# dmuley/sph-code

Hardware: AMD Instinct MI355X
Metric: particle-steps/sec + achieved HBM GB/s, 10^6-particle 3D sphere, 1/2/4/8 GPUs (higher is better)
Workload: dtype f64

## Files before the change

### include/sphx.h

```cpp
#ifndef SPHX_H
#define SPHX_H

#include <stddef.h>
#include <stdint.h>

#ifdef __cplusplus
extern "C" {
#endif

#define SPHX_OK            0
#define SPHX_E_ARG        -1
#define SPHX_E_HIP        -2
#define SPHX_E_NOMEM      -3
#define SPHX_E_STATE      -4

#define SPHX_MAX_K        64
#define SPHX_MAX_SPECIES  32

typedef struct sphx_ctx sphx_ctx;

typedef struct sphx_constants {
    double k_B;
    double amu;
    double m_h;
    double m_0;
    double dt_0;
    double max_age;
    double pos_clamp;
    double solar_luminosity;
    double c;
} sphx_constants;

typedef struct sphx_stats {
    double ms_grid;
    double ms_search;
    double ms_prep;
    double ms_density;
    double ms_pi;
    double ms_visc;
    double ms_integrate;
    double ms_total;
    int64_t n;
    int64_t steps;
    int64_t candidates;
    int64_t retries;
    int64_t cells;
    int64_t refresh_steps;
    int64_t rebuild_steps;
    double  cell_size;
    double  ms_gravity;
    int64_t fallback_queries;
    double  ms_species;
    int64_t short_rows;
    int64_t detail_steps;
    int64_t far_queries;
    int64_t outlier_levels;
    int64_t bad_accel;
    int64_t bad_energy;
    int64_t bad_state;
    int64_t bad_h;
    int64_t search_steps;
    int64_t tie_entries;
    int64_t tie_capacity;
    int64_t visc_blobs_settled;
    int64_t pi_waves_settled;
} sphx_stats;

int         sphx_create(sphx_ctx** out, int device);
void        sphx_destroy(sphx_ctx* ctx);
const char* sphx_last_error(const sphx_ctx* ctx);
int         sphx_version(void);
const char* sphx_build_info(void);
const char* sphx_tunables(const sphx_ctx* ctx);
int sphx_selftest_scan(sphx_ctx* ctx, int n, unsigned seed, long long* mismatches, int* single_launch);
int sphx_selftest_grid_order(sphx_ctx* ctx, int n, const double* x, const double* y, const double* z, double cell_size,
                             long long* mismatches, int* new_chain_taken);
int sphx_selftest_mfma_cull(sphx_ctx* ctx, double E, int blocks, unsigned seed, double* max_err_over_E2,
                            double* wrong_signs, double* kappa);
int         sphx_host_alloc(void** out, size_t bytes);
int         sphx_host_free(void* p);
int         sphx_set_constants(sphx_ctx* ctx, const sphx_constants* c);
int         sphx_get_constants(const sphx_ctx* ctx, sphx_constants* c);
int         sphx_set_tuning(sphx_ctx* ctx, double rscale, double cell_factor);
int         sphx_set_timing_detail(sphx_ctx* ctx, int on);
int         sphx_set_incremental(sphx_ctx* ctx, int verlet, double rscale_build);

int sphx_neighbors(sphx_ctx* ctx, int64_t n, int k, const double* points, double dist,
                   double eps, int64_t* idx, double* dist_out, int64_t* nontriv, double* h);

int sphx_hydro_update(sphx_ctx* ctx, int64_t n, int k, int s, const int64_t* neighbor,
                      const double* points, const double* mass, const double* sizes,
                      const double* f_un, const double* particle_type, const double* T,
                      const double* mu_array, const double* gamma_array,
                      const double* velocities, int visc_mode,
                      double* hydro_accel, double* visc_accel, double* visc_heat,
                      double* rho, double* nden, double* f_un_nb, double* rho_dust);

int sphx_density(sphx_ctx* ctx, int64_t n, int k, const double* points, const double* mass,
                 const double* particle_type, const int64_t* neighbor, double d, double* out);
int sphx_dust_density(sphx_ctx* ctx, int64_t n, int k, const double* points, const double* mass,
                      const int64_t* neighbor, const double* particle_type, const double* sizes,
                      double* out);
int sphx_num_dens(sphx_ctx* ctx, int64_t n, int k, const double* mass, const double* points,
                  const double* mu_array, const int64_t* neighbor, double d, double* out);
int sphx_del_pressure(sphx_ctx* ctx, int64_t n, int k, const double* points, const double* mass,
                      const double* particle_type, const int64_t* neighbor,
                      const double* E_internal, const double* gamma_array, double d,
                      double* out );
int sphx_artificial_viscosity(sphx_ctx* ctx, int64_t n, int k, const int64_t* neighbor,
                              const double* points, const double* particle_type,
                              const double* sizes, const double* mass, const double* densities,
                              const double* velocities, const double* T,
                              const double* gamma_array, const double* mu_array, double d,
                              double* visc_accel , double* visc_heat );
int sphx_crossing_time(sphx_ctx* ctx, int64_t n, int k, const int64_t* neighbor,
                       const double* velocities, const double* sizes,
                       const double* particle_type, double* out );
int sphx_net_impulse(sphx_ctx* ctx, int64_t n, int k, const double* points, const double* mass,
                     const double* sizes, const double* velocities, const double* particle_type,
                     const int64_t* neighbor, const double* mean_grain_mass,
                     const double* mean_cross, double* accel_onto ,
                     double* accel_reaction );

int sphx_gravity_direct(sphx_ctx* ctx, int64_t n, const double* mass, const double* points,
                        const double* sizes, double softening, double G, double* accel);

int sphx_gravity_tree(sphx_ctx* ctx, int64_t n, const double* mass, const double* points,
                      const double* sizes, double softening, double G, int ws, int k_cells,
                      double* accel);

int sphx_gravity_tree_parts(sphx_ctx* ctx, int64_t n, const double* mass, const double* points,
                            const double* sizes, double softening, double G, int ws, int k_cells, int nparts,
                            const int32_t* part_of, double* accel, int64_t* counts);

int sphx_agb_yields(sphx_ctx* ctx, int64_t n, const double* masses, const double* metallicities,
                    int nspl, const int32_t* ntx, const int32_t* nty, const double* tx,
                    const double* ty, const double* coeffs, const int32_t* mapto, double divisor,
                    int nspecies, const double* mu_specie, const double* composition,
                    double solar_mass, double* dust_out ,
                    double* gas_out );

int sphx_dt_rule(sphx_ctx* ctx, int64_t n, const double* ct, const int32_t* first, double* dt);
int sphx_clamp_arrays(sphx_ctx* ctx, int64_t n, double* points, double* velocities);
int sphx_leapfrog(sphx_ctx* ctx, int64_t n, double* points, double* velocities, double* total_accel,
                  const double* old_accel, double* E_internal, double* T, const double* mass,
                  const double* mu, const double* gamma, const double* ptype, const double* grav_accel,
                  const double* delp, const double* densities, const double* dust_densities,
                  const double* drag_on_gas, const double* drag_reaction, const double* av_accel,
                  const double* av_heat, double dt);

int sphx_state_upload(sphx_ctx* ctx, int64_t n, int s, const double* pos, const double* vel,
                      const double* mass, const double* ptype, const double* f_un,
                      const double* T, const double* mu, const double* gamma,
                      const double* E_internal, const double* accel_old);
int sphx_state_set_drag(sphx_ctx* ctx, const double* mean_grain_mass, const double* mean_cross);
int sphx_state_set_agb(sphx_ctx* ctx, int nspl, const int32_t* ntx, const int32_t* nty, const double* tx,
                       const double* ty, const double* coeffs, const int32_t* mapto, double divisor,
                       const double* mu_specie, double solar_mass);
int sphx_state_download_species(sphx_ctx* ctx, double* F, double* Z, double* agb_dust);
int sphx_state_set_loop_forms(sphx_ctx* ctx, int on, double d);
int sphx_set_clip_grad(sphx_ctx* ctx, int on);
int sphx_set_visc_mode(sphx_ctx* ctx, int mode);
int sphx_state_set_gravity(sphx_ctx* ctx, int mode, double G);
int sphx_set_gravity_order(sphx_ctx* ctx, int order);
int sphx_step(sphx_ctx* ctx, int nsteps, int k, double dist, int first, double fixed_dt);
int sphx_state_download(sphx_ctx* ctx, double* pos, double* vel, double* accel,
                        double* E_internal, double* T, double* sizes, double* rho,
                        double* nden, double* visc_heat, double* dt_last);
int sphx_state_download_pressure(sphx_ctx* ctx, double* pressure);
int sphx_arb_fields(sphx_ctx* ctx, int64_t n, const double* points, const double* mass,
                    const double* particle_type, const double* sizes, const double* T, const double* n_part,
                    const double* value, double d, int64_t m, const double* arb_points, double radius,
                    double* density, double* dust_density, double* temperature, double* dust_temperature,
                    double* photoionization, int64_t* count, int64_t* candidates, int64_t ball_id);
int sphx_arb_fields_list(sphx_ctx* ctx, int64_t n, const double* points, const double* mass,
                         const double* particle_type, const double* sizes, const double* T, const double* n_part,
                         const double* value, double d, int64_t m, const double* arb_points,
                         const int64_t* row_start, const int64_t* members, double* density, double* dust_density,
                         double* temperature, double* dust_temperature, double* photoionization, int64_t* count,
                         int64_t* candidates);
int sphx_state_sample(sphx_ctx* ctx, double d, const double* n_part, const double* value, int64_t m,
                      const double* arb_points, double radius, double* density, double* dust_density,
                      double* temperature, double* dust_temperature, double* photoionization, int64_t* count,
                      int64_t* candidates);
int sphx_arb_last_timing(sphx_ctx* ctx, double ms[4]);
#define SPHX_RAD_LINE        0
#define SPHX_RAD_SEGMENT     1
#define SPHX_RAD_TILE        256
#define SPHX_RAD_WG_RAYS     256
#define SPHX_RAD_SRC_CHUNK   16
int sphx_rad_columns(sphx_ctx* ctx, int64_t n, const double* points, const double* sizes, const double* mass,
                     const double* mu, const double* cross, int64_t n_src, const double* src, int64_t n_dst,
                     const double* dst, int mode, double* blocked , double* star_distance );
int sphx_rad_transfer(sphx_ctx* ctx, int64_t n, const double* points, const double* ptypes, const double* mass,
                      const double* sizes, const double* cross, const double* mu, int64_t n_src, const double* src,
                      const double* luminosities, int64_t n_dst, const double* dst, double dt, int mode, double* lf2,
                      double* momentum, double* extinction, double* blocked, double* star_distance, double* lum_factor);
int sphx_state_rad_transfer(sphx_ctx* ctx, const double* cross, int64_t n_src, const double* src,
                            const double* luminosities, int64_t n_dst, const double* dst, double dt, int mode, double* lf2,
                            double* momentum, double* extinction, double* blocked, double* star_distance,
                            double* lum_factor);
int sphx_rad_last_timing(sphx_ctx* ctx, double ms[4]);
#define SPHX_COOL_WG         256
int sphx_rad_cooling(sphx_ctx* ctx, int64_t n, int k, int s, const double* points, const double* ptype,
                     const double* mass, const double* f_un, const int64_t* neighbor, const double* mu, const double* T,
                     double dt, double d, double* final_comp, double* energy, double* rec_array,
                     double* row_table );
int sphx_cool_last_timing(sphx_ctx* ctx, double ms[4]);
#define SPHX_DUST_WG              256
#define SPHX_DUST_GUARD_COUNT     0
#define SPHX_DUST_GUARD_FRACTION  1
int sphx_supernova_destruction(sphx_ctx* ctx, int64_t n, int k, int s, const double* points, const double* velocities,
                               const int64_t* neighbor, const double* mass, const double* f_un, const double* mu,
                               const double* sizes, const double* densities, const double* ptype, double crit_mass,
                               double critical_density, const int32_t* species_curve ,
                               const double knots_v[8], const double knots_c[8], const double knots_si[8], int guard_mode,
                               double* frac_destruction, double* frac_reuptake, int64_t* counts );
int sphx_dust_last_timing(sphx_ctx* ctx, double ms[4]);
// ... 106 lines not shown
```

### sph-code_amd/_lib.py

```python
import ctypes as C
import os
import threading
import weakref

import numpy as np

HERE = os.path.dirname(os.path.abspath(__file__))
LIB_PATH = os.environ.get("SPHX_LIB") or os.path.join(HERE, "libsphx.so")

c_double_p = C.POINTER(C.c_double)
c_int64_p = C.POINTER(C.c_int64)
c_int32_p = C.POINTER(C.c_int32)


class SphxConstants(C.Structure):
    _fields_ = [(n, C.c_double) for n in ("k_B", "amu", "m_h", "m_0", "dt_0", "max_age", "pos_clamp", "solar_luminosity",
                                          "c")]


class SphxStats(C.Structure):
    _fields_ = [(n, C.c_double) for n in ("ms_grid", "ms_search", "ms_prep", "ms_density", "ms_pi",
                                          "ms_visc", "ms_integrate", "ms_total")] + \
               [(n, C.c_int64) for n in ("n", "steps", "candidates", "retries", "cells", "refresh_steps",
                                         "rebuild_steps")] + \
               [("cell_size", C.c_double), ("ms_gravity", C.c_double), ("fallback_queries", C.c_int64),
                ("ms_species", C.c_double), ("short_rows", C.c_int64), ("detail_steps", C.c_int64), ("far_queries", C.c_int64),
                ("outlier_levels", C.c_int64), ("bad_accel", C.c_int64), ("bad_energy", C.c_int64), ("bad_state", C.c_int64),
                ("bad_h", C.c_int64), ("search_steps", C.c_int64), ("tie_entries", C.c_int64), ("tie_capacity", C.c_int64),
                ("visc_blobs_settled", C.c_int64), ("pi_waves_settled", C.c_int64)]

    def as_dict(self):
        return {n: getattr(self, n) for n, _ in self._fields_}


SPHX_E_STATE = -4
_P = C.c_void_p
_D = c_double_p
_I = c_int64_p
SIGNATURES = {
    "sphx_create": (C.c_int, [C.POINTER(_P), C.c_int]),
    "sphx_destroy": (None, [_P]),
    "sphx_last_error": (C.c_char_p, [_P]),
    "sphx_version": (C.c_int, []),
    "sphx_build_info": (C.c_char_p, []),
    "sphx_tunables": (C.c_char_p, [_P]),
    "sphx_selftest_scan": (C.c_int, [_P, C.c_int, C.c_uint, C.POINTER(C.c_longlong), C.POINTER(C.c_int)]),
    "sphx_selftest_grid_order": (C.c_int, [_P, C.c_int, _D, _D, _D, C.c_double, C.POINTER(C.c_longlong), C.POINTER(C.c_int)]),
    "sphx_selftest_mfma_cull": (C.c_int, [_P, C.c_double, C.c_int, C.c_uint, _D, _D, _D]),
    "sphx_host_alloc": (C.c_int, [C.POINTER(_P), C.c_size_t]),
    "sphx_host_free": (C.c_int, [_P]),
    "sphx_set_constants": (C.c_int, [_P, C.POINTER(SphxConstants)]),
    "sphx_get_constants": (C.c_int, [_P, C.POINTER(SphxConstants)]),
    "sphx_set_tuning": (C.c_int, [_P, C.c_double, C.c_double]),
    "sphx_set_incremental": (C.c_int, [_P, C.c_int, C.c_double]),
    "sphx_neighbors": (C.c_int, [_P, C.c_int64, C.c_int, _D, C.c_double, C.c_double, _I, _D, _I, _D]),
    "sphx_hydro_update": (C.c_int, [_P, C.c_int64, C.c_int, C.c_int, _I] + [_D] * 9 + [C.c_int] + [_D] * 7),
    "sphx_density": (C.c_int, [_P, C.c_int64, C.c_int, _D, _D, _D, _I, C.c_double, _D]),
    "sphx_dust_density": (C.c_int, [_P, C.c_int64, C.c_int, _D, _D, _I, _D, _D, _D]),
    "sphx_num_dens": (C.c_int, [_P, C.c_int64, C.c_int, _D, _D, _D, _I, C.c_double, _D]),
    "sphx_del_pressure": (C.c_int, [_P, C.c_int64, C.c_int, _D, _D, _D, _I, _D, _D, C.c_double, _D]),
    "sphx_artificial_viscosity": (C.c_int, [_P, C.c_int64, C.c_int, _I] + [_D] * 9 + [C.c_double, _D, _D]),
    "sphx_crossing_time": (C.c_int, [_P, C.c_int64, C.c_int, _I, _D, _D, _D, _D]),
    "sphx_net_impulse": (C.c_int, [_P, C.c_int64, C.c_int, _D, _D, _D, _D, _D, _I, _D, _D, _D, _D]),
    "sphx_agb_yields": (C.c_int, [_P, C.c_int64, _D, _D, C.c_int, C.POINTER(C.c_int32), C.POINTER(C.c_int32), _D, _D, _D,
                                  C.POINTER(C.c_int32), C.c_double, C.c_int, _D, _D, C.c_double, _D, _D]),
    "sphx_dt_rule": (C.c_int, [_P, C.c_int64, _D, C.POINTER(C.c_int32), _D]),
    "sphx_clamp_arrays": (C.c_int, [_P, C.c_int64, _D, _D]),
    "sphx_leapfrog": (C.c_int, [_P, C.c_int64] + [_D] * 18 + [C.c_double]),
    "sphx_state_upload": (C.c_int, [_P, C.c_int64, C.c_int] + [_D] * 10),
    "sphx_state_set_drag": (C.c_int, [_P, _D, _D]),
    "sphx_state_set_agb": (C.c_int, [_P, C.c_int, C.POINTER(C.c_int32), C.POINTER(C.c_int32), _D, _D, _D,
                                     C.POINTER(C.c_int32), C.c_double, _D, C.c_double]),
    "sphx_state_download_species": (C.c_int, [_P, _D, _D, _D]),
    "sphx_state_set_loop_forms": (C.c_int, [_P, C.c_int, C.c_double]),
    "sphx_set_clip_grad": (C.c_int, [_P, C.c_int]),
    "sphx_set_visc_mode": (C.c_int, [_P, C.c_int]),
    "sphx_state_set_gravity": (C.c_int, [_P, C.c_int, C.c_double]),
    "sphx_set_gravity_order": (C.c_int, [_P, C.c_int]),
    "sphx_gravity_direct": (C.c_int, [_P, C.c_int64, _D, _D, _D, C.c_double, C.c_double, _D]),
    "sphx_gravity_tree": (C.c_int, [_P, C.c_int64, _D, _D, _D, C.c_double, C.c_double, C.c_int, C.c_int, _D]),
    "sphx_gravity_tree_parts": (C.c_int, [_P, C.c_int64, _D, _D, _D, C.c_double, C.c_double, C.c_int, C.c_int, C.c_int,
                                          c_int32_p, _D, _I]),
    "sphx_step": (C.c_int, [_P, C.c_int, C.c_int, C.c_double, C.c_int, C.c_double]),
    "sphx_state_download": (C.c_int, [_P] + [_D] * 10),
    "sphx_state_download_pressure": (C.c_int, [_P, _D]),
    "sphx_arb_fields": (C.c_int, [_P, C.c_int64] + [_D] * 7 + [C.c_double, C.c_int64, _D, C.c_double] + [_D] * 5 + [_I, _I, C.c_int64]),
    "sphx_arb_last_timing": (C.c_int, [_P, _D]),
    "sphx_arb_fields_list": (C.c_int, [_P, C.c_int64] + [_D] * 7 + [C.c_double, C.c_int64, _D, _I, _I] + [_D] * 5 + [_I, _I]),
    "sphx_state_sample": (C.c_int, [_P, C.c_double, _D, _D, C.c_int64, _D, C.c_double] + [_D] * 5 + [_I, _I]),
    "sphx_rad_columns": (C.c_int, [_P, C.c_int64] + [_D] * 5 + [C.c_int64, _D, C.c_int64, _D, C.c_int, _D, _D]),
    "sphx_rad_transfer": (C.c_int, [_P, C.c_int64] + [_D] * 6 + [C.c_int64, _D, _D, C.c_int64, _D, C.c_double, C.c_int] + [_D] * 6),
    "sphx_state_rad_transfer": (C.c_int, [_P, _D, C.c_int64, _D, _D, C.c_int64, _D, C.c_double, C.c_int] + [_D] * 6),
    "sphx_rad_last_timing": (C.c_int, [_P, _D]),
    "sphx_rad_cooling": (C.c_int, [_P, C.c_int64, C.c_int, C.c_int] + [_D] * 4 + [_I, _D, _D, C.c_double, C.c_double] + [_D] * 4),
    "sphx_cool_last_timing": (C.c_int, [_P, _D]),
    "sphx_supernova_destruction": (C.c_int, [_P, C.c_int64, C.c_int, C.c_int, _D, _D, _I] + [_D] * 6 + [C.c_double, C.c_double,
                                             c_int32_p, _D, _D, _D, C.c_int, _D, _D, _I]),
    "sphx_dust_last_timing": (C.c_int, [_P, _D]),
    "sphx_chemisputtering_2": (C.c_int, [_P, C.c_int64, C.c_int, C.c_int, _D, _I] + [_D] * 6 + [C.c_double, C.c_double] + [_D] * 4 +
                                         [C.c_double] * 3 + [_D, _D, _I]),
    "sphx_chem_last_timing": (C.c_int, [_P, _D]),
    "sphx_dust_bookkeeping": (C.c_int, [_P, C.c_int64, C.c_int] + [_D] * 8 + [C.c_double] + [_D] * 5 + [_I]),
    "sphx_state_dust_phase": (C.c_int, [_P, C.c_double, C.c_double] + [_D] * 5 + [C.c_double] * 5 + [c_int32_p, _D, _D, _D, C.c_int] +
                                        [_D] * 7 + [_I, _I, _D, _I]),
    "sphx_phase_last_timing": (C.c_int, [_P, _D]),
    "sphx_state_download_neighbors": (C.c_int, [_P, _I]),
    "sphx_state_download_composition": (C.c_int, [_P, _D, _D, _D, _D]),
    "sphx_state_download_drag": (C.c_int, [_P, _D, _D]),
    "sphx_get_stats": (C.c_int, [_P, C.POINTER(SphxStats)]),
    "sphx_reset_stats": (C.c_int, [_P]),
    "sphx_set_stream": (C.c_int, [_P, C.c_void_p]),
    "sphx_reset_stream": (C.c_int, [_P]),
    "sphx_sync": (C.c_int, [_P]),
    "sphx_dev_set_mean_h": (C.c_int, [_P, C.c_double]),
    "sphx_dev_search": (C.c_int, [_P, C.c_int64, C.c_int64, C.c_int, _P, _P, C.c_double, C.c_double, _P]),
    "sphx_dev_get_order": (C.c_int, [_P, C.c_int64, _P]),
    "sphx_dev_prep": (C.c_int, [_P] + [_P] * 8),
    "sphx_dev_density": (C.c_int, [_P] + [_P] * 4),
    "sphx_dev_pi": (C.c_int, [_P] + [_P] * 4),
    "sphx_dev_visc": (C.c_int, [_P] + [_P] * 4),
    "sphx_dev_visc_pairwise": (C.c_int, [_P] + [_P] * 5),
    "sphx_dev_clamp": (C.c_int, [_P, C.c_int64, _P, _P]),
    "sphx_dev_pack_rows": (C.c_int, [_P, C.c_int64, _P, C.c_int, C.POINTER(C.c_void_p), C.POINTER(C.c_int32), _P]),
    "sphx_dev_regroup": (C.c_int, [_P, C.c_int64, _P, C.c_int64, _P, C.c_int, C.POINTER(C.c_void_p),
                                   C.POINTER(C.c_int32), C.POINTER(C.c_void_p)]),
    "sphx_dev_need_map": (C.c_int, [_P, C.c_int64, _P, _P, C.POINTER(C.c_double), C.c_double, C.c_int, _P]),
    "sphx_dev_integrate_auto": (C.c_int, [_P, C.c_int64] + [_P] * 13 + [C.c_int, C.c_double, _P]),
    "sphx_dev_reach": (C.c_int, [_P, C.c_int64, _P, _P, C.c_double, C.c_double, C.c_double, _P]),
    "sphx_set_timing_detail": (C.c_int, [_P, C.c_int]),
    "sphx_dev_reach_dt": (C.c_int, [_P, C.c_int64, _P, _P, C.c_double, C.c_double, _P, _P]),
    "sphx_dev_plan_mask": (C.c_int, [_P, C.c_int64, _P, C.POINTER(C.c_double), C.c_double, C.c_int, C.c_int, C.c_int, _P, _P, _P]),
    "sphx_dev_step_scalars": (C.c_int, [_P, C.c_int64, _P, _P, C.c_double, C.c_double, _P, _P]),
    "sphx_dev_integrate": (C.c_int, [_P, C.c_int64] + [_P] * 12 + [C.c_double]),
    "sphx_dev_drag": (C.c_int, [_P] + [_P] * 6),
    "sphx_dev_set_drag_terms": (C.c_int, [_P] + [_P] * 4),
    "sphx_dev_gravity_build": (C.c_int, [_P, C.c_int64, C.c_int64, _P, _P, _D]),
    "sphx_dev_gravity_local": (C.c_int, [_P, C.c_int, C.c_double, _P, C.c_double, _P]),
    "sphx_dev_gravity_export": (C.c_int, [_P, C.c_int, C.c_int, _P, C.c_int, _P, C.c_int64, _P, C.c_int64, _P]),
    "sphx_dev_gravity_remote": (C.c_int, [_P, C.c_int64, _P, _P, C.c_int64, _P, C.c_int64, C.c_double, _P, C.c_double, _P]),
    "sphx_dev_set_gravity_accel": (C.c_int, [_P, _P]),
    "sphx_dev_set_agb": (C.c_int, [_P, C.c_int, C.c_int, C.POINTER(C.c_int32), C.POINTER(C.c_int32), _D, _D, _D,
                                   C.POINTER(C.c_int32), C.c_double, _D, C.c_double]),
    "sphx_dev_species": (C.c_int, [_P, C.c_int] + [_P] * 5),
    "sphx_dev_loop_prep": (C.c_int, [_P] + [_P] * 8 + [C.c_double]),
    "sphx_dev_loop_pass1": (C.c_int, [_P] + [_P] * 5),
    "sphx_dev_loop_pass2": (C.c_int, [_P] + [_P] * 4),
    "sphx_dev_loop_pass2_interior": (C.c_int, [_P]),
    "sphx_dev_set_reach_cap": (C.c_int, [_P, C.c_double]),
    "sphx_dev_select_blobs": (C.c_int, [_P, C.c_int]),
    "sphx_dev_blob_split_counts": (C.c_int, [_P, _P]),
    "sphx_dev_integrate_loop": (C.c_int, [_P, C.c_int64] + [_P] * 14 + [C.c_int, C.c_double, C.c_double, _P]),
}

_lib = None
_lock = threading.Lock()


def load_library():
    global _lib
    with _lock:
        if _lib is not None:
            return _lib
        if not os.path.exists(LIB_PATH):
            raise RuntimeError(
                "libsphx.so is not built (%s). Run `python -c 'import __graft_entry__ as g; g.build()'` "
                "or `python sph-code_amd/build.py`. There is no CPU fallback." % LIB_PATH)
        lib = C.CDLL(LIB_PATH)
        for name, (res, args) in SIGNATURES.items():
            fn = getattr(lib, name)
            fn.restype = res
            fn.argtypes = args
        _lib = lib
        return lib


def f64(a, shape=None):
    out = np.ascontiguousarray(a, dtype=np.float64)
    if shape is not None and out.shape != shape:
        raise ValueError("expected shape %s, got %s" % (shape, out.shape))
    return out


# ... 132 lines not shown
```

### sph-code_amd/csrc/sphx_api.hip

```cpp
#include "sphx_internal.h"
#include <stdarg.h>
#include <stdlib.h>
#include <new>

int sphx_set_err(sphx_ctx* ctx, int code, const char* fmt, ...) {
    if (ctx) {
        va_list ap;
        va_start(ap, fmt);
        vsnprintf(ctx->err, sizeof(ctx->err), fmt, ap);
        va_end(ap);
    }
    return code;
}

void sphx_release(sphx_ctx* ctx, DevBuf& b) {
    for (size_t q = 0; q < ctx->allocs.size(); ++q)
        if (ctx->allocs[q] == b.p) { ctx->allocs[q] = ctx->allocs.back(); ctx->allocs.pop_back(); break; }
    if (b.p) (void)hipFree(b.p);
    b.p = nullptr;
    b.cap = 0;
}

int sphx_ensure(sphx_ctx* ctx, DevBuf& b, size_t bytes, hipStream_t in_use_on) {
    if (bytes == 0) bytes = 8;
// ... 495 lines not shown
static int step_cell_hint(sphx_ctx* ctx, int64_t n, double* cell_hint) {
    *cell_hint = 0.0;
    if (ctx->step_count == 0) return SPHX_OK;
    const double* hs;
    if (ctx->lag_hvalid[ctx->lag_hslot]) {
        HIPCHK(hipEventSynchronize(ctx->lag_halias[ctx->lag_hslot] ? ctx->lag_halias[ctx->lag_hslot]
                                                                     : ctx->lag_hev[ctx->lag_hslot]));
        hs = ctx->pinned->lag[ctx->lag_hslot].hs;
        const u64* sv = (const u64*)hs;
        for (int q = 0; q < 10; ++q) ctx->knn_lag[q] = sv[(SC_NFAILQ - SC_HSUM) + q];
        ctx->knn_lag_valid = true;
    } else {
        HIPCHK(hipMemcpyAsync(ctx->pinned->hsum, ctx->scal.as<double>() + SC_HSUM, sizeof(ctx->pinned->hsum),
                              hipMemcpyDeviceToHost, ctx->stream));
        HIPCHK(hipStreamSynchronize(ctx->stream));
        hs = ctx->pinned->hsum;
    }
    const double hmean = hs[3] > 0.0 ? hs[0] / hs[3] : 0.0;
    if (hmean > 0.0 && isfinite(hmean)) {
        *cell_hint = ctx->cell_factor * sphx_cell_feedback(ctx, n) * hmean;
        ctx->h_clip = ctx->h_clip_factor * hmean;
    }
    return SPHX_OK;
}

static int step_search(sphx_ctx* ctx, int k, double dist, hipEvent_t* ev) {
    const int64_t n = ctx->n;
    if (ctx->use_verlet) SPHX_TRY(sphx_clamp(ctx, n, ctx->st));
    SPHX_TRY(sphx_ensure(ctx, ctx->nbr, (size_t)k * ctx->npad * sizeof(int)));
    if (ctx->use_verlet && ctx->list_valid && ctx->list_n == n && ctx->list_k == k) {
        StateArrays& r = ctx->st;
        HIPCHK(hipEventRecord(ev[1], ctx->stream));
        int64_t nfail = 0;
        SPHX_TRY(sphx_knn_refresh(ctx, n, k, r.x.as<double>(), r.y.as<double>(), r.z.as<double>(),
                                  ctx->nbr.as<int>(), r.hprev.as<double>(), &nfail));
        if (nfail == 0) {
            ctx->stats.refresh_steps++;
            return SPHX_OK;
        }
        ctx->list_valid = false;
    }
    double cell_hint = 0.0;
    SPHX_TRY(step_cell_hint(ctx, n, &cell_hint));
    {
        StateArrays& r = ctx->st;
        const bool blob = ctx->use_blob && !ctx->use_verlet;
        GridBuildOpts g;
        g.lagged = true;
        g.alias_ev = ev[1];
        g.sort_cells_later = blob;
        g.count_curve = blob && ctx->side_stream && ctx->ev_perm;
        if (!ctx->use_verlet) { g.clamp_vel[0] = r.vx.as<double>(); g.clamp_vel[1] = r.vy.as<double>(); g.clamp_vel[2] = r.vz.as<double>(); }
        SPHX_TRY(sphx_build_grid(ctx, n, k, r.x.as<double>(), r.y.as<double>(), r.z.as<double>(), cell_hint, g));
        if (blob) SPHX_TRY(sphx_build_blob_order(ctx, n, true));
    }
    const bool split = ctx->side_stream && !ctx->use_verlet;
    SPHX_TRY(sphx_permute_state(ctx, n, split, ev[1]));
    StateArrays& r = ctx->st;
    KnnIn in;
    in.xs = r.x.as<double>(); in.ys = r.y.as<double>(); in.zs = r.z.as<double>();
    in.id = r.id.as<int>(); in.inv = ctx->inv.as<int>();
    in.rsearch = r.hprev.as<double>();
    in.hinted = ctx->step_count > 0 && !ctx->use_verlet;
    in.lag_external = true;
    in.rscale = ctx->rscale;
    in.rbound = dist;
    KnnOut o;
    o.nbr = ctx->nbr.as<int>();
    o.h_sorted = r.hprev.as<double>();
    o.idx64 = nullptr; o.dist = nullptr; o.nontriv = nullptr; o.h_by_id = nullptr;
    if (ctx->use_verlet) {
        SPHX_TRY(sphx_ensure(ctx, ctx->list64, (size_t)n * 64 * sizeof(int)));
        SPHX_TRY(sphx_ensure(ctx, ctx->dref, (size_t)n * sizeof(double)));
        o.list64 = ctx->list64.as<int>();
        o.dref = ctx->dref.as<double>();
        in.rscale = ctx->rscale_build;
    }
    SPHX_TRY(sphx_knn(ctx, n, k, in, o));
    if (split) HIPCHK(hipStreamWaitEvent(ctx->stream, ctx->ev_perm, 0));
    if (ctx->use_verlet) {
        SPHX_TRY(sphx_save_list_positions(ctx, n, r.x.as<double>(), r.y.as<double>(), r.z.as<double>()));
        ctx->list_valid = true;
        ctx->list_n = n;
        ctx->list_k = k;
    }
    ctx->stats.rebuild_steps++;
    return SPHX_OK;
}

static int step_h_sums_out(sphx_ctx* ctx, int64_t n, const double* h, hipStream_t stream) {
    SPHX_TRY(sphx_hsum(ctx, n, h, stream));
    const int hsl = ctx->lag_hslot ^ 1;
    HIPCHK(hipMemcpyAsync(ctx->pinned->lag[hsl].hs, ctx->scal.as<double>() + SC_HSUM,
                          (SC_KGDBG + 2 - SC_HSUM + 1) * sizeof(double), hipMemcpyDeviceToHost, stream));
    HIPCHK(hipEventRecord(ctx->lag_hev[hsl], stream));
    ctx->lag_halias[hsl] = nullptr;
    ctx->lag_hvalid[hsl] = true;
    ctx->lag_hslot = hsl;
    return SPHX_OK;
}

static int step_sums(sphx_ctx* ctx, int k, hipEvent_t* ev, hipEvent_t search_end, bool detail) {
    const int64_t n = ctx->n;
    StateArrays& s = ctx->st;
    const bool pairwise = ctx->visc_mode == 1 && !ctx->loop_forms;
    const bool fork = ctx->qorder && ctx->use_lds && !ctx->loop_forms && ctx->side_stream;
    if (fork) HIPCHK(hipStreamWaitEvent(ctx->side_stream, search_end, 0));
    else SPHX_TRY(step_h_sums_out(ctx, n, s.hprev.as<double>(), ctx->stream));
    if (ctx->qorder && ctx->use_lds) SPHX_TRY(sphx_blob_translate(ctx, n, k));
    const bool species = ctx->s > 0 && ctx->fun_id.p;
    if (ctx->loop_forms) {
        if (ctx->drag || species)
            SPHX_TRY(sphx_prep(ctx, n, prep_in_of_state(s), pairwise, ctx->stream));
        if (detail) HIPCHK(hipEventRecord(ev[3], ctx->stream));
        SPHX_TRY(sphx_loop_step_sums(ctx, n, k, ctx->loop_d));
        if (detail) HIPCHK(hipEventRecord(ev[9], ctx->stream));
        if (species) SPHX_TRY(sphx_step_species(ctx, n, k));
        if (detail) HIPCHK(hipEventRecord(ev[4], ctx->stream));
        if (detail) HIPCHK(hipEventRecord(ev[5], ctx->stream));
    } else {
        SPHX_TRY(sphx_prep(ctx, n, prep_in_of_state(s), pairwise, fork ? ctx->side_stream : ctx->stream));
        if (fork) {
            HIPCHK(hipEventRecord(ctx->ev_join, ctx->side_stream));
            HIPCHK(hipStreamWaitEvent(ctx->stream, ctx->ev_join, 0));
            SPHX_TRY(step_h_sums_out(ctx, n, s.hprev.as<double>(), ctx->side_stream));
        }
        if (detail) HIPCHK(hipEventRecord(ev[3], ctx->stream));
        const bool sp_fused = species && ctx->species_fused && ctx->species_lds && ctx->use_lds && ctx->qorder && ctx->blob_lists &&
                              !ctx->map_perm && ctx->sp == 16 && ctx->s <= 16 && k <= SPHX_MAX_K;
        if (sp_fused) {
            const int S = ctx->s;
            SPHX_TRY(sphx_ensure(ctx, ctx->rho, (size_t)n * sizeof(double)));
            SPHX_TRY(sphx_ensure(ctx, ctx->rhod, (size_t)n * sizeof(double)));
            SPHX_TRY(sphx_ensure(ctx, ctx->nden, (size_t)n * sizeof(double)));
            SPHX_TRY(sphx_ensure(ctx, ctx->G, (size_t)n * 3 * sizeof(double)));
            SPHX_TRY(sphx_ensure(ctx, ctx->ha, (size_t)n * 3 * sizeof(double)));
            SPHX_TRY(sphx_ensure(ctx, ctx->F, (size_t)n * S * sizeof(double)));
            if (ctx->agb_on) {
                SPHX_TRY(sphx_ensure(ctx, ctx->Zmet, (size_t)n * sizeof(double)));
                SPHX_TRY(sphx_ensure(ctx, ctx->agb_dust, (size_t)n * S * sizeof(double)));
            }
            SPHX_TRY(sphx_blob_density_species(ctx, n, k, true, S, ctx->fun_id.as<double>(), s.id.as<int>(),
                                               s.m.as<double>(), ctx->F.as<double>(), ctx->Zmet.as<double>(),
                                               ctx->agb_dust.as<double>(), (ctx->agb_on && ctx->Zmet.p && ctx->agb_dust.p) ? 1 : 0));
        } else {
            SPHX_TRY(sphx_pass_density(ctx, n, k, true));
        }
        if (detail) HIPCHK(hipEventRecord(ev[9], ctx->stream));
        if (species && !sp_fused) SPHX_TRY(sphx_step_species(ctx, n, k));
        if (detail) HIPCHK(hipEventRecord(ev[4], ctx->stream));
        if (ctx->visc_mode == 1) {
            SPHX_TRY(sphx_pass_visc_pw(ctx, n, k, s.m.as<double>()));
        } else {
            SPHX_TRY(sphx_pass_pi(ctx, n, k, s.hprev.as<double>(), s.ptype.as<double>()));
            if (detail) HIPCHK(hipEventRecord(ev[5], ctx->stream));
            SPHX_TRY(sphx_pass_visc(ctx, n, k, s.m.as<double>()));
        }
    }
    if (ctx->drag)
        SPHX_TRY(sphx_pass_drag(ctx, n, k, s.m.as<double>(), s.ptype.as<double>(), s.mgm.as<double>(), s.mcs.as<double>()));
    return SPHX_OK;
}

static int one_step(sphx_ctx* ctx, int k, double dist, int first, double fixed_dt, bool call_first, bool call_last) {
    const int64_t n = ctx->n;
    const int ring = (int)(ctx->step_count % 3);
    hipEvent_t* ev = ctx->evring[ring];
    const bool detail = ctx->timing_detail;
    ctx->ev_detail[ring] = detail;
    const bool rec0 = detail || call_first, rec7 = detail || call_last;
    ctx->ev_has07[ring] = (rec0 ? 1 : 0) | (rec7 ? 2 : 0) | (ctx->visc_mode == 1 && !ctx->loop_forms ? 4 : 0);
    ctx->map_perm = nullptr;
    ctx->qorder = nullptr;
    ctx->blob_lists = false;
    ctx->blob_split_valid = false;
    ctx->pass_part = 0;
    ctx->nbr_api_valid = false;
    sphx_step_list_drop(ctx);
    if (rec0) HIPCHK(hipEventRecord(ev[0], ctx->stream));
    SPHX_TRY(step_search(ctx, k, dist, ev));
    HIPCHK(hipEventRecord(ev[2], ctx->stream));
    SPHX_TRY(step_sums(ctx, k, ev, ev[2], detail));
    if (detail) HIPCHK(hipEventRecord(ev[6], ctx->stream));
    StateArrays& s = ctx->st;
    if (ctx->gravity) {
        SPHX_TRY(sphx_ensure(ctx, ctx->grav, (size_t)n * 3 * sizeof(double)));
        double* eps = ctx->scal.as<double>() + SC_GRAV_EPS;
        SPHX_TRY(sphx_median(ctx, n, s.hprev.as<double>(), eps));
        if (ctx->gravity == 1)
            SPHX_TRY(sphx_gravity_launch(ctx, n, s.x.as<double>(), s.y.as<double>(), s.z.as<double>(), 1,
                                         s.m.as<double>(), eps, 0.0, ctx->grav_G, nullptr, ctx->grav.as<double>()));
        else
            SPHX_TRY(sphx_gravity_tree_launch(ctx, n, s.x.as<double>(), s.y.as<double>(), s.z.as<double>(),
                                              s.m.as<double>(), ctx->grav_ws, eps, 0.0, ctx->grav_G, nullptr,
                                              ctx->grav.as<double>()));
    }
    if (detail) HIPCHK(hipEventRecord(ev[8], ctx->stream));
    SPHX_TRY(sphx_integrate(ctx, n, 1, first, fixed_dt));
    if (rec7) HIPCHK(hipEventRecord(ev[7], ctx->stream));
    ctx->step_count++;
    return SPHX_OK;
}

static int collect_stats(sphx_ctx* ctx, int ring) {
    if (!(ctx->ev_pending & (1u << ring))) return SPHX_OK;
    ctx->ev_pending &= ~(1u << ring);
    hipEvent_t* ev = ctx->evring[ring];
    const int has = ctx->ev_has07[ring];
    HIPCHK(hipEventSynchronize((has & 2) ? ev[7] : ev[2]));
    sphx_stats& st = ctx->stats;
    float ms[7] = {0.f, 0.f, 0.f, 0.f, 0.f, 0.f, 0.f};
    HIPCHK(hipEventElapsedTime(&ms[1], ev[1], ev[2]));
    st.ms_search += ms[1];
    st.steps += 1;
    st.search_steps += 1;
    st.n = ctx->n;
    if (!ctx->ev_detail[ring]) return SPHX_OK;
    float tot;
    HIPCHK(hipEventElapsedTime(&tot, ev[0], ev[7]));
    HIPCHK(hipEventElapsedTime(&ms[0], ev[0], ev[1]));
    st.ms_grid += ms[0]; st.ms_total += tot;
    for (int i = 2; i < 6; ++i) {
        if ((has & 4) && i >= 4) break;
        HIPCHK(hipEventElapsedTime(&ms[i], ev[i], ev[i + 1]));
    }
    if (has & 4) HIPCHK(hipEventElapsedTime(&ms[5], ev[4], ev[6]));
    st.ms_prep += ms[2];
    float mg = 0.f, mi = 0.f;
    HIPCHK(hipEventElapsedTime(&mg, ev[6], ev[8]));
    HIPCHK(hipEventElapsedTime(&mi, ev[8], ev[7]));
    ms[6] = mi;
    st.ms_gravity += mg;
    {
        float md = 0.f, msp = 0.f;
        HIPCHK(hipEventElapsedTime(&md, ev[3], ev[9]));
        HIPCHK(hipEventElapsedTime(&msp, ev[9], ev[4]));
        ms[3] = md;
        st.ms_species += msp;
    }
    st.ms_density += ms[3]; st.ms_pi += ms[4]; st.ms_visc += ms[5]; st.ms_integrate += ms[6];
    st.detail_steps += 1;
    return SPHX_OK;
}

extern "C" int sphx_step(sphx_ctx* ctx, int nsteps, int k, double dist, int first, double fixed_dt) {
    if (!ctx) return SPHX_E_ARG;
    if (!ctx->has_state) return sphx_set_err(ctx, SPHX_E_STATE, "sphx_step before sphx_state_upload");
    if (k < 1 || k > SPHX_MAX_K) return sphx_set_err(ctx, SPHX_E_ARG, "N_NEIGH=%d not in 1..%d", k, SPHX_MAX_K);
    if (nsteps < 1) return sphx_set_err(ctx, SPHX_E_ARG, "nsteps=%d < 1", nsteps);
    HIPCHK(hipSetDevice(ctx->device));
    if (!(dist > 0.0) || !isfinite(dist)) dist = 0.0;
    ctx->k = k;
    const bool per_call = !ctx->timing_detail;
    if (per_call) HIPCHK(hipEventRecord(ctx->ev[8], ctx->stream));
    for (int it = 0; it < nsteps; ++it) {
        const int ring = (int)(ctx->step_count % 3);
        SPHX_TRY(collect_stats(ctx, ring));
        SPHX_TRY(one_step(ctx, k, dist, first && it == 0, fixed_dt, false, false));
        ctx->ev_pending |= 1u << ring;
        SPHX_TRY(collect_stats(ctx, (ring + 1) % 3));
    }
    ctx->step_list_valid = true; ctx->step_qorder = ctx->qorder; ctx->step_list_n = ctx->n; ctx->step_list_k = k;
    if (per_call) HIPCHK(hipEventRecord(ctx->ev[9], ctx->stream));
    HIPCHK(hipMemcpyAsync(ctx->pinned->scal, ctx->scal.p, SC_NSLOTS * 8, hipMemcpyDeviceToHost, ctx->stream));
    HIPCHK(hipStreamSynchronize(ctx->stream));
    for (int r = 0; r < 3; ++r) SPHX_TRY(collect_stats(ctx, (int)((ctx->step_count + r) % 3)));
    if (per_call) {
        float tot = 0.f;
        HIPCHK(hipEventElapsedTime(&tot, ctx->ev[8], ctx->ev[9]));
        ctx->stats.ms_total += tot;
    }
    const u64* sc = ctx->pinned->scal;
    memcpy(&ctx->dt_last, &sc[SC_DT], sizeof(double));
    ctx->stats.candidates = (int64_t)sc[SC_CAND];
    ctx->stats.retries = (int64_t)sc[SC_RETRY];
    ctx->stats.fallback_queries = (int64_t)(u32)sc[SC_NFAILQ];
    ctx->stats.short_rows = (int64_t)sc[SC_SHORT];
    SPHX_TRY(sphx_badc_read(ctx));
    return SPHX_OK;
}

extern "C" int sphx_state_download(sphx_ctx* ctx, double* pos, double* vel, double* accel,
                                   double* E_internal, double* T, double* sizes, double* rho,
                                   double* nden, double* visc_heat, double* dt_last) {
    if (!ctx) return SPHX_E_ARG;
    if (!ctx->has_state) return sphx_set_err(ctx, SPHX_E_STATE, "no state uploaded");
    HIPCHK(hipSetDevice(ctx->device));
    const int64_t n = ctx->n;
    const size_t nb = (size_t)n * sizeof(double);
    StateArrays& s = ctx->st;
    const int* id = s.id.as<int>();
    SPHX_TRY(sphx_ensure(ctx, ctx->out_a, 3 * nb));
    double* stage = ctx->out_a.as<double>();
    struct V3 { double* host; DevBuf *a, *b, *c; };
    V3 v3[] = {{pos, &s.x, &s.y, &s.z}, {vel, &s.vx, &s.vy, &s.vz}, {accel, &s.ax, &s.ay, &s.az}};
    for (V3& v : v3) {
        if (!v.host) continue;
        SPHX_TRY(sphx_soa3_to_aos_by_id(ctx, n, id, v.a->as<double>(), v.b->as<double>(), v.c->as<double>(), stage));
        SPHX_TRY(download(ctx, v.host, stage, 3 * nb));
        HIPCHK(hipStreamSynchronize(ctx->stream));
    }
    struct V1 { double* host; const double* dev; };
    const bool stepped = ctx->step_count > 0;
    V1 v1[] = {{E_internal, s.E.as<double>()}, {T, s.T.as<double>()}, {sizes, s.hprev.as<double>()},
               {rho, stepped ? ctx->rho.as<double>() : nullptr},
               {nden, stepped ? ctx->nden.as<double>() : nullptr},
               {visc_heat, stepped ? ctx->vh.as<double>() : nullptr}};
    for (V1& v : v1) {
        if (!v.host) continue;
        if (!v.dev) { memset(v.host, 0, nb); continue; }
        SPHX_TRY(sphx_scatter_rows_by_id(ctx, n, 1, id, v.dev, stage));
        SPHX_TRY(download(ctx, v.host, stage, nb));
        HIPCHK(hipStreamSynchronize(ctx->stream));
    }
    if (dt_last) *dt_last = ctx->dt_last;
    return SPHX_OK;
}

int sphx_agb_table_set(sphx_ctx* ctx, int S, int nspl, const int32_t* ntx, const int32_t* nty, const double* tx, const double* ty,
                       const double* coeffs, const int32_t* mapto, double divisor, const double* mu_specie, double solar_mass) {
    ctx->agb_on = false;
    if (nspl == 0) return SPHX_OK;
    if (S < 7 || S > AGB_MAX_SPEC) return sphx_set_err(ctx, SPHX_E_ARG, "AGB table: %d species (7..%d)", S, AGB_MAX_SPEC);
    if (!ntx || !nty || !tx || !ty || !coeffs || !mapto || !mu_specie)
        return sphx_set_err(ctx, SPHX_E_ARG, "AGB table: NULL argument");
    if (nspl < 1 || nspl > AGB_MAX_SPL) return sphx_set_err(ctx, SPHX_E_ARG, "AGB table: %d splines", nspl);
    if (!(divisor != 0.0)) return sphx_set_err(ctx, SPHX_E_ARG, "AGB table: divisor is 0");
    HIPCHK(hipSetDevice(ctx->device));
    AgbTable& t = ctx->agb;
    t.nspl = nspl; t.nspec = S;
    size_t ntx_tot = 0, nty_tot = 0, nc_tot = 0;
    for (int o = 0; o < nspl; ++o) {
        if (ntx[o] < 4 || nty[o] < 4) return sphx_set_err(ctx, SPHX_E_ARG, "AGB table: spline %d has fewer than 4 knots", o);
        if (mapto[o] < 0 || mapto[o] >= S) return sphx_set_err(ctx, SPHX_E_ARG, "AGB table: mapto[%d]=%d out of range", o, mapto[o]);
        ntx_tot += ntx[o]; nty_tot += nty[o]; nc_tot += (size_t)(ntx[o] - 2) * (nty[o] - 2);
    }
    size_t ox = 0, oy = ntx_tot, oc = ntx_tot + nty_tot;
    for (int o = 0; o < nspl; ++o) {
        t.tx_off[o] = (int)ox; t.ty_off[o] = (int)oy; t.c_off[o] = (int)oc;
        t.ntx[o] = ntx[o]; t.nty[o] = nty[o]; t.mapto[o] = mapto[o];
        ox += ntx[o]; oy += nty[o]; oc += (size_t)(ntx[o] - 2) * (nty[o] - 2);
    }
    for (int s = 0; s < S; ++s) t.mu[s] = mu_specie[s];
    t.divisor = divisor; t.solar = solar_mass;
    SPHX_TRY(sphx_ensure(ctx, ctx->agb_knots, (ntx_tot + nty_tot + nc_tot + 6 * (size_t)nspl) * sizeof(double)));
    double* kd = ctx->agb_knots.as<double>();
    {
        double meta[6 * AGB_MAX_SPL];
        t.covered = 0u;
        for (int o = 0; o < nspl; ++o) {
            bool later = false;
            for (int o2 = o + 1; o2 < nspl; ++o2) later = later || mapto[o2] == mapto[o];
            meta[6 * o + 0] = t.tx_off[o]; meta[6 * o + 1] = t.ty_off[o]; meta[6 * o + 2] = t.c_off[o];
            meta[6 * o + 3] = t.ntx[o]; meta[6 * o + 4] = t.nty[o]; meta[6 * o + 5] = later ? -1.0 : (double)mapto[o];
            t.covered |= 1u << mapto[o];
        }
        t.meta_off = (int)(ntx_tot + nty_tot + nc_tot);
        HIPCHK(hipMemcpyAsync(kd + t.meta_off, meta, 6 * (size_t)nspl * sizeof(double), hipMemcpyHostToDevice, ctx->stream));
        HIPCHK(hipStreamSynchronize(ctx->stream));
    }
    HIPCHK(hipMemcpyAsync(kd, tx, ntx_tot * sizeof(double), hipMemcpyHostToDevice, ctx->stream));
    HIPCHK(hipMemcpyAsync(kd + ntx_tot, ty, nty_tot * sizeof(double), hipMemcpyHostToDevice, ctx->stream));
    HIPCHK(hipMemcpyAsync(kd + ntx_tot + nty_tot, coeffs, nc_tot * sizeof(double), hipMemcpyHostToDevice, ctx->stream));
    HIPCHK(hipStreamSynchronize(ctx->stream));
    t.knots = kd;
    ctx->agb_on = true;
    return SPHX_OK;
}

extern "C" int sphx_state_set_agb(sphx_ctx* ctx, int nspl, const int32_t* ntx, const int32_t* nty, const double* tx,
                                  const double* ty, const double* coeffs, const int32_t* mapto, double divisor,
                                  const double* mu_specie, double solar_mass) {
    if (!ctx) return SPHX_E_ARG;
    if (!ctx->has_state) return sphx_set_err(ctx, SPHX_E_STATE, "sphx_state_set_agb before sphx_state_upload");
    ctx->agb_on = false;
    if (nspl == 0) return SPHX_OK;
    if (ctx->s < 7 || !ctx->fun_id.p)
        return sphx_set_err(ctx, SPHX_E_STATE, "sphx_state_set_agb: the state carries no composition (f_un) of >= 7 species");
    return sphx_agb_table_set(ctx, ctx->s, nspl, ntx, nty, tx, ty, coeffs, mapto, divisor, mu_specie, solar_mass);
}

__global__ __launch_bounds__(256) void scatter_species_major(int n, int S, const int* id, const double* in, double* out) {
    const int t = blockIdx.x * blockDim.x + threadIdx.x;
    if (t >= n) return;
    const size_t o = (size_t)id[t];
    for (int s = 0; s < S; ++s) out[(size_t)s * n + o] = in[(size_t)s * n + t];
}
extern "C" int sphx_state_download_species(sphx_ctx* ctx, double* F, double* Z, double* agb_dust) {
    if (!ctx) return SPHX_E_ARG;
    if (!ctx->has_state || ctx->s < 1 || !ctx->fun_id.p || ctx->step_count < 1)
        return sphx_set_err(ctx, SPHX_E_STATE, "sphx_state_download_species: no species pass has run (state without f_un, "
                                                 "or no step yet)");
    if ((Z || agb_dust) && !ctx->agb_on) return sphx_set_err(ctx, SPHX_E_STATE, "sphx_state_download_species: no AGB table set");
    HIPCHK(hipSetDevice(ctx->device));
    const int64_t n = ctx->n;
    const int S = ctx->s;
    const int* id = ctx->st.id.as<int>();
    SPHX_TRY(sphx_ensure(ctx, ctx->out_a, (size_t)n * S * sizeof(double)));
    double* stage = ctx->out_a.as<double>();
    if (F) {
        hipLaunchKernelGGL(scatter_species_major, dim3((unsigned)((n + 255) / 256)), dim3(256), 0, ctx->stream, (int)n, S, id,
                           ctx->F.as<double>(), stage);
        SPHX_TRY(download(ctx, F, stage, (size_t)n * S * sizeof(double)));
        HIPCHK(hipStreamSynchronize(ctx->stream));
    }
    if (Z) {
        SPHX_TRY(sphx_scatter_rows_by_id(ctx, n, 1, id, ctx->Zmet.as<double>(), stage));
        SPHX_TRY(download(ctx, Z, stage, (size_t)n * sizeof(double)));
        HIPCHK(hipStreamSynchronize(ctx->stream));
    }
    if (agb_dust) {
        SPHX_TRY(sphx_scatter_rows_by_id(ctx, n, S, id, ctx->agb_dust.as<double>(), stage));
        SPHX_TRY(download(ctx, agb_dust, stage, (size_t)n * S * sizeof(double)));
        HIPCHK(hipStreamSynchronize(ctx->stream));
    }
    return SPHX_OK;
}

int sphx_badc_read(sphx_ctx* ctx) {
    u64* hb = ctx->pinned->badc;
    HIPCHK(hipMemcpyAsync(hb, ctx->badc.p, (size_t)BADC_BUCKETS * BADC_STRIDE * sizeof(u64), hipMemcpyDeviceToHost, ctx->stream));
    HIPCHK(hipStreamSynchronize(ctx->stream));
    u64 tot[4] = {0, 0, 0, 0};
    for (int b = 0; b < BADC_BUCKETS; ++b)
        for (int q = 0; q < 4; ++q) tot[q] += hb[b * BADC_STRIDE + q];
    ctx->stats.bad_accel = (int64_t)tot[BAD_ACCEL]; ctx->stats.bad_energy = (int64_t)tot[BAD_ENERGY];
    ctx->stats.bad_state = (int64_t)tot[BAD_STATE]; ctx->stats.bad_h = (int64_t)tot[BAD_H];
    return SPHX_OK;
}

extern "C" int sphx_get_stats(sphx_ctx* ctx, sphx_stats* out) {
    if (!ctx || !out) return SPHX_E_ARG;
    SPHX_TRY(sphx_dev_collect(ctx));
    if (ctx->map_perm) {
        HIPCHK(hipSetDevice(ctx->device));
        SPHX_TRY(sphx_badc_read(ctx));
    }
    ctx->stats.tie_entries = 0;
    ctx->stats.tie_capacity = ctx->tie_cap_last;
    if (ctx->tie_count_dev) {
        int cnt = 0;
        u64 nfail = 0;
        HIPCHK(hipSetDevice(ctx->device));
        HIPCHK(hipMemcpyAsync(&cnt, ctx->tie_count_dev, sizeof(int), hipMemcpyDeviceToHost, ctx->stream));
        HIPCHK(hipMemcpyAsync(&nfail, ctx->scal.as<u64>() + SC_NFAILQ, sizeof(u64), hipMemcpyDeviceToHost, ctx->stream));
        HIPCHK(hipStreamSynchronize(ctx->stream));
        ctx->stats.tie_entries = (int64_t)(u32)cnt;
        if (ctx->map_perm) ctx->stats.fallback_queries = (int64_t)(u32)nfail;
    }
    if (ctx->scal.p) {
        u64 cnt[2] = {0, 0};
        HIPCHK(hipSetDevice(ctx->device));
        HIPCHK(hipMemcpyAsync(cnt, ctx->scal.as<u64>() + SC_SETTLED, sizeof(cnt), hipMemcpyDeviceToHost, ctx->stream));
        HIPCHK(hipStreamSynchronize(ctx->stream));
        ctx->stats.visc_blobs_settled = (int64_t)cnt[0];
        ctx->stats.pi_waves_settled = (int64_t)cnt[1];
    }
    *out = ctx->stats;
    for (int w = 0; w < 2; ++w) {
        if (!ctx->lbs_state[w].p) continue;
        int flag = 0;
        HIPCHK(hipSetDevice(ctx->device));
        HIPCHK(hipMemcpy(&flag, ctx->lbs_state[w].as<int>() + 2, sizeof(int), hipMemcpyDeviceToHost));
        if (flag) return sphx_set_err(ctx, SPHX_E_STATE, "lookback_scan_kernel: a tile's sum never arrived (results since then are wrong)");
    }
    return SPHX_OK;
}
extern "C" int sphx_set_timing_detail(sphx_ctx* ctx, int on) {
    if (!ctx) return SPHX_E_ARG;
    ctx->timing_detail = on != 0;
    return SPHX_OK;
}

extern "C" int sphx_reset_stats(sphx_ctx* ctx) {
    if (!ctx) return SPHX_E_ARG;
    SPHX_TRY(sphx_dev_collect(ctx));
    memset(&ctx->stats, 0, sizeof(ctx->stats));
    HIPCHK(hipMemsetAsync(ctx->scal.as<u64>() + SC_CAND, 0, 2 * sizeof(u64), ctx->stream));
    HIPCHK(hipMemsetAsync(ctx->scal.as<u64>() + SC_SHORT, 0, sizeof(u64), ctx->stream));
    HIPCHK(hipMemsetAsync(ctx->scal.as<u64>() + SC_SETTLED, 0, 2 * sizeof(u64), ctx->stream));
    HIPCHK(hipMemsetAsync(ctx->badc.p, 0, (size_t)BADC_BUCKETS * BADC_STRIDE * sizeof(u64), ctx->stream));
    HIPCHK(hipStreamSynchronize(ctx->stream));
    return SPHX_OK;
}
```

### sph-code_amd/csrc/sphx_blob.h

```cpp
#pragma once
#include "sphx_internal.h"
#include "sphx_pair.h"
#include "sphx_settled.h"

#ifndef BLOB_P
#define BLOB_P 128
#endif
#define BLOB_T (2 * BLOB_P)
#define LPP SPHX_SUM_PARTS
#define PASS_T (BLOB_P * LPP)
#ifndef BLOB_S
#define BLOB_S 960
#endif
#ifndef DEDUP_PRIO
#define DEDUP_PRIO 2
#endif
#ifndef BLOB_STAGE_PRIO
#define BLOB_STAGE_PRIO 1
#endif
#ifndef PASS_MINW
#define PASS_MINW 4
#endif
#define BLOB_PROBES 96
#define SLOT_NONE 0xFFFFu
// ... 5 lines not shown
__device__ __forceinline__ Q4 lload4(const double2* img, int s, int c2) {
    const double2 lo = img[(2 * c2) * BLOB_S + s];
    const double2 hi = img[(2 * c2 + 1) * BLOB_S + s];
    return Q4{lo.x, lo.y, hi.x, hi.y};
}
struct Q8 { Q4 lo, hi; };
__device__ __forceinline__ Q8 lload8(const double2* img, int s) { return Q8{lload4(img, s, 0), lload4(img, s, 1)}; }
template <class Rec>
__device__ __forceinline__ Q8 gload8(const Rec* r) {
    const double* q = reinterpret_cast<const double*>(r);
    return Q8{gload4(q), gload4(q + 4)};
}
__device__ __forceinline__ double sqrt_mid(double x) {
    const double y = __builtin_amdgcn_rsq(x);
    double g = x * y;
    double h = 0.5 * y;
    const double r = __builtin_fma(-h, g, 0.5);
    g = __builtin_fma(g, r, g);
    h = __builtin_fma(h, r, h);
    const double d0 = __builtin_fma(-g, g, x);
    g = __builtin_fma(d0, h, g);
    const double d1 = __builtin_fma(-g, g, x);
    g = __builtin_fma(d1, h, g);
    return x > 0.0 ? g : 0.0;
}
struct SqrtMid { __device__ __forceinline__ double operator()(double x) const { return sqrt_mid(x); } };

__device__ __forceinline__ double pair_swap(double v) {
    const long long b = __double_as_longlong(v);
    const int lo = __builtin_amdgcn_update_dpp(0, (int)b, 0xB1, 0xF, 0xF, true);
    const int hi = __builtin_amdgcn_update_dpp(0, (int)(b >> 32), 0xB1, 0xF, 0xF, true);
    return __longlong_as_double(((long long)hi << 32) | (unsigned)lo);
}
__device__ __forceinline__ double pair_swap2(double v) {
    const long long b = __double_as_longlong(v);
    const int lo = __builtin_amdgcn_update_dpp(0, (int)b, 0x4E, 0xF, 0xF, true);
    const int hi = __builtin_amdgcn_update_dpp(0, (int)(b >> 32), 0x4E, 0xF, 0xF, true);
    return __longlong_as_double(((long long)hi << 32) | (unsigned)lo);
}
__device__ __forceinline__ double group_total(double acc) {
    acc = acc + pair_swap(acc);
    if (LPP == 4) acc = acc + pair_swap2(acc);
    return acc;
}
__device__ __forceinline__ double group_max(double v) {
    v = fmax(v, pair_swap(v));
    if (LPP == 4) v = fmax(v, pair_swap2(v));
    return v;
}
template <class S>
__device__ __forceinline__ void group_total_fields(S& s) {
    constexpr int NF = sizeof(S) / sizeof(double);
    static_assert(sizeof(S) == NF * sizeof(double), "a struct of doubles");
    double f[NF];
    __builtin_memcpy(f, &s, sizeof(S));
#pragma unroll
    for (int q = 0; q < NF; ++q) f[q] = group_total(f[q]);
    __builtin_memcpy(&s, f, sizeof(S));
}

#define NSTAGE ((BLOB_S + PASS_T - 1) / PASS_T)
#define NB (8 / LPP)
#define KPAD(k) ((((k) + 7) / 8) * 8)
#define IMG_BYTES(per_slot, k) ((size_t)BLOB_S * (per_slot) + (size_t)KPAD(k) * BLOB_P * sizeof(u16))

template <int NSIDE, class Rec>
__device__ __forceinline__ void stage(double2* img, double* side, u16* tile, const Rec* __restrict__ rec,
                                      const double* __restrict__ g0, int g0_stride,
                                      const double* __restrict__ g1, int g1_stride,
                                      const int* __restrict__ uq, const u16* __restrict__ slot16, int npad,
                                      int k, int b) {
    __builtin_amdgcn_s_setprio(BLOB_STAGE_PRIO);
    int ju[NSTAGE];
#pragma unroll
    for (int r = 0; r < NSTAGE; ++r) {
        const int s = threadIdx.x + r * PASS_T;
        ju[r] = (s < BLOB_S) ? uq[s] : -1;
    }
    const int pieces = KPAD(k) * (BLOB_P / 8);
    for (int q = threadIdx.x; q < pieces; q += PASS_T) {
        const int kk = q / (BLOB_P / 8), c = q % (BLOB_P / 8);
        uint4 v = make_uint4(0xFFFFFFFFu, 0xFFFFFFFFu, 0xFFFFFFFFu, 0xFFFFFFFFu);
        if (kk < k) v = *reinterpret_cast<const uint4*>(slot16 + (size_t)kk * npad + (size_t)b * BLOB_P + c * 8);
        *reinterpret_cast<uint4*>(tile + kk * BLOB_P + c * 8) = v;
    }
    double2 c[NSTAGE][4];
    double e0[NSTAGE], e1[NSTAGE];
#pragma unroll
    for (int r = 0; r < NSTAGE; ++r) {
        const int j = ju[r] < 0 ? 0 : ju[r];
        const double2* g = reinterpret_cast<const double2*>(&rec[j]);
        c[r][0] = g[0]; c[r][1] = g[1]; c[r][2] = g[2]; c[r][3] = g[3];
        e0[r] = (NSIDE > 0) ? g0[(size_t)j * g0_stride] : 0.0;
        e1[r] = (NSIDE > 1) ? g1[(size_t)j * g1_stride] : 0.0;
    }
#pragma unroll
    for (int r = 0; r < NSTAGE; ++r) {
        const int s = threadIdx.x + r * PASS_T;
        if (ju[r] >= 0) {
            if (NSIDE == 2) c[r][3].y = e0[r];
            img[0 * BLOB_S + s] = c[r][0]; img[1 * BLOB_S + s] = c[r][1];
            img[2 * BLOB_S + s] = c[r][2]; img[3 * BLOB_S + s] = c[r][3];
            if (NSIDE == 1) side[s] = e0[r];
            if (NSIDE == 2) side[s] = e1[r];
        }
    }
    __builtin_amdgcn_s_setprio(0);
}

__device__ __forceinline__ void load_slots(unsigned (&sl)[NB], const u16* tile, int m0, int half, int t) {
#pragma unroll
    for (int u = 0; u < NB; ++u) sl[u] = tile[(LPP * (m0 + u) + half) * BLOB_P + t];
}
__device__ __forceinline__ bool all_staged(const unsigned (&sl)[NB]) {
    unsigned worst = sl[0];
#pragma unroll
    for (int u = 1; u < NB; ++u) worst = worst > sl[u] ? worst : sl[u];
    return __ballot(worst >= SLOT_OVER) == 0ull;
}


struct BlobSel { const int* list; const int* cnt; int mode; };
__device__ __forceinline__ int blob_sel_count(const BlobSel& s, int nblk) {
    if (!s.list) return nblk;
    return (s.mode == 1) ? s.cnt[0] : (s.mode == 2) ? s.cnt[1] : s.cnt[0] + s.cnt[1];
}
__device__ __forceinline__ int blob_sel_at(const BlobSel& s, int bi, int count) {
    const int q = xcd_block(bi, count);
    return s.list ? s.list[q + (s.mode == 2 ? s.cnt[0] : 0)] : q;
}
BlobSel sphx_blob_sel(sphx_ctx* ctx, int part);

int sphx_blob_grid(sphx_ctx* ctx, int nblk);
int sphx_lds_opt_in(sphx_ctx* ctx, const void* kernel, size_t bytes);

#define BLOB_KERNEL __global__ __launch_bounds__(PASS_T, PASS_MINW) void
#define BLOB_COMMON int n, int npad, int k, int nblk, const int* __restrict__ nbr, const u16* __restrict__ slot16, \
                    const int* __restrict__ uniq, const int* __restrict__ qorder
template <class Kern, class... Rest>
static int blob_launch(sphx_ctx* ctx, Kern kern, int per_slot, size_t extra, int64_t n, int k, Rest... rest) {
    const int64_t npad = sphx_pad64(n);
    const int nblk = (int)((npad + BLOB_P - 1) / BLOB_P);
    SPHX_TRY(sphx_lds_opt_in(ctx, reinterpret_cast<const void*>(kern), IMG_BYTES(per_slot, SPHX_MAX_K) + extra));
    hipLaunchKernelGGL(kern, dim3(sphx_blob_grid(ctx, nblk)), dim3(PASS_T), IMG_BYTES(per_slot, k) + extra, ctx->stream, (int)n,
                       (int)npad, k, nblk, ctx->nbr.as<int>(), ctx->slot16.as<u16>(), ctx->uniq.as<int>(), ctx->qorder, rest...);
    HIPCHK(hipGetLastError());
    return SPHX_OK;
}

template <class P, class = void> struct BlobSettles { static constexpr bool value = false; };
template <class P> struct BlobSettles<P, decltype((void)P::SETTLES)> { static constexpr bool value = P::SETTLES; };
template <class P, class = void> struct BlobSaturates { static constexpr bool value = false; };
template <class P> struct BlobSaturates<P, decltype((void)P::SATURATES)> { static constexpr bool value = P::SATURATES; };
enum { BLOB_CNT_BLOBS_SETTLED = 0, BLOB_CNT_WAVES_SATURATED = 1 };
struct BlobSides { const double* g0 = nullptr; int s0 = 0; const double* g1 = nullptr; int s1 = 0; };

template <int NSIDE>
struct BlobLds {
    static __device__ __forceinline__ double2* img() { extern __shared__ double2 img[]; return img; }
    static __device__ __forceinline__ double* side() { return reinterpret_cast<double*>(img() + 4 * BLOB_S); }
    static __device__ __forceinline__ u16* tile() { return reinterpret_cast<u16*>(side() + (NSIDE ? BLOB_S : 0)); }
};

template <bool FAST, bool CLIP, class P>
__device__ __forceinline__ void blob_batch(const P& ps, typename P::Sums& a, double (&out)[NB], const unsigned (&sl)[NB],
                                           const int* __restrict__ jp, size_t colstep, const typename P::Row& row) {
    typedef BlobLds<P::NSIDE> L;
    typename P::Nb f[NB];
#pragma unroll
    for (int u = 0; u < NB; ++u) {
        if (FAST || sl[u] < SLOT_OVER) f[u] = ps.staged(L::img(), L::side(), (int)sl[u], jp + u * colstep);
        else if (sl[u] == SLOT_OVER) f[u] = ps.global(jp[u * colstep]);
        else f[u] = P::none(row);
    }
    if (FAST) __builtin_amdgcn_sched_barrier(0);
#pragma unroll
    for (int u = 0; u < NB; ++u) {
        out[u] = 0.0;
        if (!FAST && sl[u] == SLOT_NONE) continue;
        out[u] = ps.template term<CLIP>(a, f[u], row);
    }
}
template <class P>
__device__ __forceinline__ void blob_batch_any(const P& ps, int clip, typename P::Sums& a, double (&out)[NB],
                                               const unsigned (&sl)[NB], const int* __restrict__ jp, size_t colstep,
                                               const typename P::Row& row) {
    const bool fast = all_staged(sl);
    if constexpr (P::CLIPS) {
        if (fast && !clip) blob_batch<true, false>(ps, a, out, sl, jp, colstep, row);
        else if (fast) blob_batch<true, true>(ps, a, out, sl, jp, colstep, row);
        else if (!clip) blob_batch<false, false>(ps, a, out, sl, jp, colstep, row);
        else blob_batch<false, true>(ps, a, out, sl, jp, colstep, row);
    } else {
        if (fast) blob_batch<true, false>(ps, a, out, sl, jp, colstep, row);
        else blob_batch<false, false>(ps, a, out, sl, jp, colstep, row);
    }
}
template <bool FAST, class P>
__device__ __forceinline__ void blob_batch_short(const P& ps, double (&out)[NB], const unsigned (&sl)[NB],
                                                 const int* __restrict__ jp, size_t colstep, const typename P::Row& row) {
    typedef BlobLds<P::NSIDE> L;
    typename P::Vel f[NB];
#pragma unroll
    for (int u = 0; u < NB; ++u) {
        if (FAST || sl[u] < SLOT_OVER) f[u] = P::short_staged(L::img(), (int)sl[u]);
        else if (sl[u] == SLOT_OVER) f[u] = ps.short_global(jp[u * colstep]);
        else f[u] = P::short_none(row);
    }
#pragma unroll
    for (int u = 0; u < NB; ++u) {
        out[u] = 0.0;
        if (!FAST && sl[u] == SLOT_NONE) continue;
        out[u] = P::term_short(f[u], row);
    }
}
struct RowAhead { int i, o; unsigned first; double own; };
template <class P>
__device__ __forceinline__ RowAhead blob_row_ahead(const P& ps, int i, int p, int n, const u16* __restrict__ slot16,
                                                   const int* __restrict__ omap) {
    RowAhead r;
    r.i = i;
    r.o = (p < n) ? (omap ? omap[i] : i) : 0x7FFFFFFF;
    r.first = (p < n) ? slot16[p] : SLOT_NONE;
    r.own = ps.own(i);
    return r;
}
template <int T>
__device__ __forceinline__ bool block_all_at_barrier(bool mine, unsigned round) {
    __shared__ int verdict[2][T / 64];
    static_assert(T / 64 == 8, "eight waves: read as two 16-B pieces");
    int* v = verdict[round & 1];
    const int wave_all = __ballot(!mine) == 0ull;
    if ((threadIdx.x & 63) == 0) v[threadIdx.x >> 6] = wave_all;
    __syncthreads();
    const int4 lo = *reinterpret_cast<const int4*>(v), hi = *reinterpret_cast<const int4*>(v + 4);
    const int all = (lo.x & lo.y) & (lo.z & lo.w) & (hi.x & hi.y) & (hi.z & hi.w);
    return __builtin_amdgcn_readfirstlane(all) != 0;
}
template <int T>
__device__ __forceinline__ void block_add_count(unsigned v, u64* dst) {
    __shared__ unsigned sm[T / 64];
    if ((threadIdx.x & 63) == 0) sm[threadIdx.x >> 6] = v;
    __syncthreads();
    if (threadIdx.x == 0) {
        unsigned r = 0;
        for (int w = 0; w < T / 64; ++w) r += sm[w];
        if (r) atomicAdd(dst, (u64)r);
    }
}
template <class P>
__device__ __forceinline__ void blob_row_point(const P& ps, typename P::Row& row, const int* __restrict__ nbr, int p,
                                               int t) {
    typedef BlobLds<P::NSIDE> L;
    const unsigned sl0 = L::tile()[t];
    if (sl0 < SLOT_OVER) P::row_point(row, ps.staged(L::img(), L::side(), (int)sl0, nbr + p));
    else if (sl0 == SLOT_OVER) P::row_point(row, ps.global(nbr[p]));
}

template <class P>
__device__ __forceinline__ void blob_pass(const P& ps, int n, int npad, int k, int nblk, const int* __restrict__ nbr,
                                          const u16* __restrict__ slot16, const int* __restrict__ uniq,
                                          const int* __restrict__ qorder, int clip, const int* __restrict__ omap,
                                          int n_active, u64* ct_bits, const BlobSel& sel, u64* counts = nullptr) {
    static_assert(P::PER_SLOT == 64 + (P::NSIDE ? 8 : 0), "image bytes per slot: the record and one side value");
    constexpr bool SETTLES = BlobSettles<P>::value, SATURATES = BlobSaturates<P>::value;
    static_assert(!SATURATES || LPP == 4, "sphx_wave_saturated: a row's lanes are one nibble of the wave's mask");
    typedef BlobLds<P::NSIDE> L;
    const BlobSides sd = ps.sides();
    const int t = threadIdx.x / LPP, half = threadIdx.x & (LPP - 1);
    u64 my_ct = SPHX_CT_NONE;
    unsigned blobs_settled = 0, waves_saturated = 0;
    const int nsel = blob_sel_count(sel, nblk);
    const int stride = gridDim.x;
    auto particle_of = [&](int bq) -> int {
        const int pq = blob_sel_at(sel, bq, nsel) * BLOB_P + t;
        return (pq < n) ? qorder[pq] : 0;
    };
    auto nothing_left = [&](const RowAhead& r) -> bool {
        return !(r.o < n_active) || sphx_row_settled(r.own, r.first != SLOT_NONE, true);
    };
    RowAhead cur{0, 0x7FFFFFFF, SLOT_NONE, 0.0};
    int i_next = 0;
    bool blob_settled = false;
    unsigned round = 0;
    if constexpr (SETTLES) {
        if ((int)blockIdx.x < nsel)
            cur = blob_row_ahead(ps, particle_of(blockIdx.x), blob_sel_at(sel, blockIdx.x, nsel) * BLOB_P + t, n, slot16, omap);
        if ((int)blockIdx.x + stride < nsel) i_next = particle_of(blockIdx.x + stride);
        blob_settled = block_all_at_barrier<PASS_T>(nothing_left(cur), round++);
    }
    for (int bi = blockIdx.x; bi < nsel; bi += stride) {
        const int b = blob_sel_at(sel, bi, nsel);
        const int p = b * BLOB_P + t;
        int i, o;
        bool settled = false;
        auto fetch_ahead = [&]() {
            if constexpr (SETTLES) {
                if (bi + stride < nsel) {
                    cur = blob_row_ahead(ps, i_next, blob_sel_at(sel, bi + stride, nsel) * BLOB_P + t, n, slot16, omap);
                    if (bi + 2 * stride < nsel) i_next = particle_of(bi + 2 * stride);
                }
            }
        };
        if constexpr (SETTLES) {
            i = cur.i; o = cur.o;
            settled = sphx_row_settled(cur.own, cur.first != SLOT_NONE, o < n_active);
            if (blob_settled) {
                fetch_ahead();
                if (settled && !half) ps.settle(o);
                ++blobs_settled;
                blob_settled = block_all_at_barrier<PASS_T>(nothing_left(cur), round++);
                continue;
            }
        } else {
            i = (p < n) ? qorder[p] : 0;
        }
        stage<P::NSIDE>(L::img(), L::side(), L::tile(), ps.rec, sd.g0, sd.s0, sd.g1, sd.s1, uniq + (size_t)b * BLOB_S,
                        slot16, npad, k, b);
        typename P::Row row = ps.load_row(i);
        if constexpr (!SETTLES) o = (p < n) ? (omap ? omap[i] : i) : 0x7FFFFFFF;
        ps.load_out(row, o, o < n_active);
        if constexpr (SETTLES) fetch_ahead();
        __syncthreads();
        if (o < n_active) {
            if (SETTLES && __ballot(!settled) == 0ull) {
                if constexpr (SETTLES) { if (!half) ps.settle(o); }
            } else {
                if constexpr (P::ROW_FROM_LIST) blob_row_point(ps, row, nbr, p, t);
                typename P::Sums a{};
                double mx = 0.0;
                if (P::wanted(row)) {
                    const int nm = KPAD(k) / LPP;
                    unsigned sl[NB];
                    load_slots(sl, L::tile(), 0, half, t);
                    bool short_form = false;
                    bool short_used = false;
                    for (int m0 = 0; m0 < nm; m0 += NB) {
                        unsigned cur_sl[NB];
#pragma unroll
                        for (int u = 0; u < NB; ++u) cur_sl[u] = sl[u];
                        if (m0 + NB < nm) load_slots(sl, L::tile(), m0 + NB, half, t);
                        double out[NB];
                        const int* jp = nbr + ((size_t)(LPP * m0 + half) * npad + p);
                        if constexpr (SATURATES) {
                            if (__builtin_expect(short_form, false)) {
                                short_used = true;
                                if (all_staged(cur_sl)) blob_batch_short<true>(ps, out, cur_sl, jp, LPP * (size_t)npad, row);
                                else blob_batch_short<false>(ps, out, cur_sl, jp, LPP * (size_t)npad, row);
                            } else {
                                blob_batch_any(ps, clip, a, out, cur_sl, jp, LPP * (size_t)npad, row);
                                short_form = sphx_wave_saturated(__ballot(P::saturated(a)), __ballot(true));
                            }
                        } else {
                            blob_batch_any(ps, clip, a, out, cur_sl, jp, LPP * (size_t)npad, row);
                        }
                        if (P::VOTES) {
#pragma unroll
                            for (int u = 0; u < NB; ++u) mx = fmax(mx, out[u]);
                        }
                    }
                    if (SATURATES && short_used) ++waves_saturated;
                }
                group_total_fields(a);
                if (P::VOTES) mx = group_max(mx);
                if (!half) {
                    const u64 cb = ps.finish(a, mx, row, i, o);
                    my_ct = cb < my_ct ? cb : my_ct;
                }
            }
        }
        if constexpr (SETTLES) blob_settled = block_all_at_barrier<PASS_T>(nothing_left(cur), round++);
        else __syncthreads();
    }
    if (P::VOTES) block_min_vote<PASS_T>(my_ct, ct_bits);
    if constexpr (SETTLES) {
        if (counts && threadIdx.x == 0 && blobs_settled) atomicAdd(counts + BLOB_CNT_BLOBS_SETTLED, (u64)blobs_settled);
    }
    if constexpr (SATURATES) {
        if (counts) block_add_count<PASS_T>(waves_saturated, counts + BLOB_CNT_WAVES_SATURATED);
    }
}
```

### sph-code_amd/csrc/sphx_blob.hip

```cpp
#include "sphx_blob.h"
#include "sphx_wave.h"
#pragma clang fp contract(off)
#include <float.h>
#include <stdlib.h>
#include <stdio.h>
#ifndef BLOB_PI_SATURATES
#define BLOB_PI_SATURATES 1
#endif

#define DD_TAB 2048
#define DD_PROBES 64
__device__ __forceinline__ unsigned dd_hash(int j) { return ((unsigned)j * 2654435761u) >> 21; }

__global__ __launch_bounds__(BLOB_T) void blob_dedup_kernel(int n, int npad, int k, int slots,
                                                            const int* __restrict__ nbr, u16* slot16,
                                                            int* uniq, const int* __restrict__ qorder,
                                                            const int* __restrict__ omap, int n_active,
                                                            unsigned char* bclass) {
    __builtin_amdgcn_s_setprio(DEDUP_PRIO);
    extern __shared__ u16 dd_tile[];
    __shared__ int key[DD_TAB];
    __shared__ u16 slot_of[DD_TAB];
    __shared__ int wave_tot[BLOB_T / 64];
    const int b = xcd_block(blockIdx.x, gridDim.x);
// ... 61 lines not shown
    __syncthreads();
    constexpr int EPT = DD_TAB / BLOB_T;
    const int e0 = threadIdx.x * EPT;
    int cnt = 0;
#pragma unroll
    for (int q = 0; q < EPT; ++q) cnt += key[e0 + q] != -1;
    const int incl = wave_scan_incl(cnt);
    const int lane = threadIdx.x & 63, wv = threadIdx.x >> 6;
    if (lane == 63) wave_tot[wv] = incl;
    __syncthreads();
    int base = incl - cnt, total = 0;
#pragma unroll
    for (int w = 0; w < BLOB_T / 64; ++w) {
        const int tw = wave_tot[w];
        if (w < wv) base += tw;
        total += tw;
    }
    int* uq = uniq + (size_t)b * BLOB_S;
    int needs_ghost = 0;
#pragma unroll
    for (int q = 0; q < EPT; ++q) {
        const int j = key[e0 + q];
        if (j != -1) {
            slot_of[e0 + q] = (u16)(base < slots ? base : SLOT_OVER);
            if (base < slots) uq[base] = j;
            ++base;
            if (bclass && omap[j] >= n_active) needs_ghost = 1;
        }
    }
    for (int q = (total < slots ? total : slots) + threadIdx.x; q < BLOB_S; q += BLOB_T) uq[q] = -1;
    __syncthreads();
    const int pieces = k * (BLOB_P / 8);
    for (int q = threadIdx.x; q < pieces; q += BLOB_T) {
        u16* src = dd_tile + q * 8;
        const int kk = q / (BLOB_P / 8), c = q % (BLOB_P / 8);
        unsigned v[8];
#pragma unroll
        for (int u = 0; u < 8; ++u) {
            const unsigned e = src[u];
            v[u] = e < DD_TAB ? (unsigned)slot_of[e] : e;
            if (v[u] == SLOT_OVER) needs_ghost = 1;
        }
        if ((size_t)b * BLOB_P + c * 8 < (size_t)npad)
            *reinterpret_cast<uint4*>(slot16 + (size_t)kk * npad + (size_t)b * BLOB_P + c * 8) =
                make_uint4(v[0] | (v[1] << 16), v[2] | (v[3] << 16), v[4] | (v[5] << 16), v[6] | (v[7] << 16));
    }
    if (bclass) {
        const int owned_q = (half == 0 && p < n && omap[qorder[p]] < n_active) ? 1 : 0;
        const int any_owned = __syncthreads_or(owned_q);
        const int any_ghost = __syncthreads_or(needs_ghost);
        if (threadIdx.x == 0) bclass[b] = (unsigned char)(!any_owned ? 2 : (any_ghost ? 1 : 0));
    }
}

#define SPLIT_T 1024
__global__ __launch_bounds__(SPLIT_T) void blob_split_kernel(int nblk, const unsigned char* __restrict__ bclass, int* list,
                                                             int* cnt) {
    __shared__ int wsum[2][SPLIT_T / 64];
    const int per = (nblk + SPLIT_T - 1) / SPLIT_T;
    const int b0 = threadIdx.x * per, b1 = (b0 + per < nblk) ? b0 + per : nblk;
    int c0 = 0, c1 = 0;
    for (int b = b0; b < b1; ++b) { const int c = bclass[b]; c0 += c == 0; c1 += c == 1; }
    const int i0 = wave_scan_incl(c0), i1 = wave_scan_incl(c1);
    const int lane = threadIdx.x & 63, wv = threadIdx.x >> 6;
    if (lane == 63) { wsum[0][wv] = i0; wsum[1][wv] = i1; }
    __syncthreads();
    int o0 = i0 - c0, o1 = i1 - c1, t0 = 0, t1 = 0;
    for (int w = 0; w < SPLIT_T / 64; ++w) {
        if (w < wv) { o0 += wsum[0][w]; o1 += wsum[1][w]; }
        t0 += wsum[0][w]; t1 += wsum[1][w];
    }
    for (int b = b0; b < b1; ++b) {
        const int c = bclass[b];
        if (c == 0) list[o0++] = b;
        else if (c == 1) list[t0 + o1++] = b;
    }
    if (threadIdx.x == 0) { cnt[0] = t0; cnt[1] = t1; cnt[2] = nblk - t0 - t1; }
}

int sphx_blob_translate(sphx_ctx* ctx, int64_t n, int k) {
    const int64_t npad = sphx_pad64(n);
    const int nblk = (int)((npad + BLOB_P - 1) / BLOB_P);
    SPHX_TRY(sphx_ensure(ctx, ctx->slot16, (size_t)k * npad * sizeof(u16) + 512));
    SPHX_TRY(sphx_ensure(ctx, ctx->uniq, (size_t)nblk * BLOB_S * sizeof(int)));
    int slots = ctx->blob_slots;
    if (slots < 1) slots = 1;
    if (slots > BLOB_S) slots = BLOB_S;
    const bool split = ctx->map_perm != nullptr && ctx->blob_split_on;
    unsigned char* bclass = nullptr;
    ctx->blob_split_valid = false;
    if (split) {
        SPHX_TRY(sphx_ensure(ctx, ctx->blob_class, (size_t)nblk));
        SPHX_TRY(sphx_ensure(ctx, ctx->blob_split, ((size_t)nblk + 4) * sizeof(int)));
        bclass = ctx->blob_class.as<unsigned char>();
    }
    hipLaunchKernelGGL(blob_dedup_kernel, dim3(nblk), dim3(BLOB_T), (size_t)k * BLOB_P * sizeof(u16), ctx->stream, (int)n, (int)npad, k, slots,
                       ctx->nbr.as<int>(), ctx->slot16.as<u16>(), ctx->uniq.as<int>(), ctx->qorder, ctx->map_perm,
                       ctx->map_nactive, bclass);
    if (split) {
        int* list = ctx->blob_split.as<int>();
        hipLaunchKernelGGL(blob_split_kernel, dim3(1), dim3(SPLIT_T), 0, ctx->stream, nblk, bclass, list, list + (size_t)nblk);
        ctx->blob_split_valid = true;
        ctx->blob_split_nblk = nblk;
    }
    HIPCHK(hipGetLastError());
    ctx->blob_lists = true;
    return SPHX_OK;
}


struct DensityPass {
    typedef RecA Rec;
    typedef DensAcc Sums;
    static constexpr int NSIDE = 0, PER_SLOT = 64;
    static constexpr bool CLIPS = true, VOTES = false, ROW_FROM_LIST = true;
    const RecA* __restrict__ rec;
    double *rho_s, *rho, *rhod, *nden, *G, *ha;
    struct Row { double xr, yr, zr, hi2, ci, Ai; };
    typedef Q8 Nb;
    __device__ __forceinline__ BlobSides sides() const { return {}; }
    __device__ __forceinline__ Row load_row(int i) const {
        const Q8 s = gload8(&rec[i]);
        return Row{s.lo.a, s.lo.b, s.lo.c, s.lo.d, -6.0 * s.hi.a, s.hi.c};
    }
    __device__ __forceinline__ static void load_out(Row&, int, bool) {}
    __device__ __forceinline__ static void row_point(Row& r, const Nb& f) { r.xr = f.lo.a; r.yr = f.lo.b; r.zr = f.lo.c; }
    __device__ __forceinline__ static bool wanted(const Row&) { return true; }
    __device__ __forceinline__ Nb staged(const double2* img, const double*, int s, const int*) const {
        return lload8(img, s);
    }
    __device__ __forceinline__ Nb global(int j) const { return gload8(&rec[j]); }
    __device__ __forceinline__ static Nb none(const Row& r) { return Nb{Q4{r.xr, r.yr, r.zr, 0.0}, Q4{0.0, 0.0, 0.0, 0.0}}; }
    template <bool CLIP>
    __device__ __forceinline__ double term(Sums& a, const Nb& f, const Row& r) const {
        return density_term<SqrtMid>(a, f.lo, f.hi, r.xr, r.yr, r.zr, r.hi2, r.ci, r.Ai, CLIP);
    }
    __device__ __forceinline__ u64 finish(const Sums& a, double, const Row&, int i, int o) const {
        rho[o] = a.rho; rhod[o] = a.rd; nden[o] = a.n;
        rho_s[i] = a.rho;
        if (G) { G[3 * (size_t)o + 0] = -a.gx; G[3 * (size_t)o + 1] = -a.gy; G[3 * (size_t)o + 2] = -a.gz; }
        ha[3 * (size_t)o + 0] = -a.gx / a.rho;
        ha[3 * (size_t)o + 1] = -a.gy / a.rho;
        ha[3 * (size_t)o + 2] = -a.gz / a.rho;
        return SPHX_CT_NONE;
    }
};
BLOB_KERNEL blob_density_kernel(BLOB_COMMON, int clip, const int* __restrict__ omap, int n_active,
                                const RecA* __restrict__ rec, double* rho_s, double* rho, double* rhod, double* nden,
                                double* G, double* ha, BlobSel sel) {
    blob_pass(DensityPass{rec, rho_s, rho, rhod, nden, G, ha}, n, npad, k, nblk, nbr, slot16, uniq, qorder, clip, omap,
              n_active, nullptr, sel);
}

struct PiPass {
    typedef RecB Rec;
    struct Sums { double pi; };
    static constexpr int NSIDE = 1, PER_SLOT = 72;
    static constexpr bool CLIPS = false, VOTES = true, ROW_FROM_LIST = true;
    static constexpr bool SATURATES = BLOB_PI_SATURATES != 0;
    const RecB* __restrict__ rec;
    const double* __restrict__ rho_s;
    const RecSelf* __restrict__ selfr;
    RecBC* bc;
    double *Pi, *BwOut;
    struct Row { Q4 r0, rv; double rho_i, cs_i, ms_i, h_i; };
    struct Nb { Q8 q; double rho; };
    __device__ __forceinline__ BlobSides sides() const { return {rho_s, 1}; }
    __device__ __forceinline__ Row load_row(int i) const {
        const RecSelf sf = selfr[i];
        const Q8 s = gload8(&rec[i]);
        return Row{s.lo, s.hi, rho_s[i], sf.csi, sf.mg, sf.h};
    }
    __device__ __forceinline__ static void load_out(Row&, int, bool) {}
    __device__ __forceinline__ static void row_point(Row& r, const Nb& f) { r.r0 = f.q.lo; r.rv = f.q.hi; }
    __device__ __forceinline__ static bool wanted(const Row&) { return true; }
    __device__ __forceinline__ Nb staged(const double2* img, const double* side, int s, const int*) const {
        return Nb{lload8(img, s), side[s]};
    }
    __device__ __forceinline__ Nb global(int j) const { return Nb{gload8(&rec[j]), rho_s[j]}; }
    __device__ __forceinline__ static Nb none(const Row& r) { return Nb{Q8{r.r0, r.rv}, r.rho_i}; }
    template <bool CLIP>
    __device__ __forceinline__ double term(Sums& a, const Nb& f, const Row& r) const {
        const PiPair t = pi_term<SqrtMid>(f.q.lo, f.q.hi, f.rho, r.r0, r.rv, r.rho_i, r.cs_i);
        a.pi += t.pi;
        return t.rel;
    }
    typedef Q4 Vel;
    __device__ __forceinline__ static bool saturated(const Sums& a) { return sphx_is_nan(a.pi); }
    __device__ __forceinline__ static Vel short_staged(const double2* img, int s) { return lload4(img, s, 1); }
    __device__ __forceinline__ Vel short_global(int j) const { return gload4(reinterpret_cast<const double*>(&rec[j]) + 4); }
    __device__ __forceinline__ static Vel short_none(const Row& r) { return r.rv; }
    __device__ __forceinline__ static double term_short(const Vel& qv, const Row& r) { return pi_rel(qv, r.rv); }
    __device__ __forceinline__ u64 finish(const Sums& a, double maxrel, const Row& r, int i, int o) const {
        Pi[o] = a.pi;
        const double bw = fmax(r.ms_i, 0.0) * a.pi;
        bc[i].Bw = bw;
        if (BwOut) BwOut[o] = bw;
        return (r.ms_i > 0.0) ? ct_vote_bits(r.h_i, maxrel) : SPHX_CT_NONE;
    }
};
BLOB_KERNEL blob_pi_kernel(BLOB_COMMON, const int* __restrict__ omap, int n_active, const RecB* __restrict__ recb,
                           const double* __restrict__ rho_s, const RecSelf* __restrict__ selfr, RecBC* bc, double* Pi,
                           double* BwOut, u64* ct_bits, BlobSel sel, u64* counts) {
    blob_pass(PiPass{recb, rho_s, selfr, bc, Pi, BwOut}, n, npad, k, nblk, nbr, slot16, uniq, qorder, 0, omap, n_active,
              ct_bits, sel, counts);
}

struct ViscPass {
    typedef RecB Rec;
    typedef ViscAcc Sums;
    static constexpr int NSIDE = 2, PER_SLOT = 72;
    static constexpr bool CLIPS = true, VOTES = false, ROW_FROM_LIST = true;
    static constexpr bool SETTLES = true;
    const RecB* __restrict__ rec;
    const RecBC* __restrict__ bc;
    const double* __restrict__ m;
    double *va, *vh;
    struct Row { Q4 r0, rv; double hi2, ci, Bi, mi; };
    struct Nb { Q8 q; double c1; };
    __device__ __forceinline__ BlobSides sides() const {
        const double* bcd = reinterpret_cast<const double*>(bc);
        return {bcd, 2, bcd + 1, 2};
    }
    __device__ __forceinline__ Row load_row(int i) const {
        const double2 bci = *reinterpret_cast<const double2*>(&bc[i]);
        const Q8 s = gload8(&rec[i]);
        return Row{s.lo, s.hi, s.lo.d, -6.0 * bci.y, bci.x, 0.0};
    }
    __device__ __forceinline__ void load_out(Row& r, int o, bool on) const { r.mi = on ? m[o] : 0.0; }
    __device__ __forceinline__ static void row_point(Row& r, const Nb& f) { r.r0 = f.q.lo; r.rv = f.q.hi; }
    __device__ __forceinline__ static bool wanted(const Row&) { return true; }
    __device__ __forceinline__ Nb staged(const double2* img, const double* side, int s, const int*) const {
        return Nb{lload8(img, s), side[s]};
    }
    __device__ __forceinline__ Nb global(int j) const {
        Nb f{gload8(&rec[j]), 0.0};
        const double2 tt = *reinterpret_cast<const double2*>(&bc[j]);
        f.q.hi.d = tt.x; f.c1 = tt.y;
        return f;
    }
    __device__ __forceinline__ static Nb none(const Row& r) { return Nb{Q8{r.r0, r.rv}, 0.0}; }
    template <bool CLIP>
    __device__ __forceinline__ double term(Sums& a, const Nb& f, const Row& r) const {
        visc_term<SqrtMid>(a, f.q.lo, f.q.hi, f.q.hi.d, f.c1, r.r0, r.rv, r.hi2, r.ci, r.Bi, CLIP);
        return 0.0;
    }
    __device__ __forceinline__ u64 finish(const Sums& a, double, const Row& r, int, int o) const {
        va[3 * (size_t)o + 0] = -a.x; va[3 * (size_t)o + 1] = -a.y; va[3 * (size_t)o + 2] = -a.z;
        vh[o] = a.h * r.mi / 2.0;
        return SPHX_CT_NONE;
    }
    __device__ __forceinline__ double own(int i) const { return bc[i].Bw; }
    __device__ __forceinline__ void settle(int o) const {
        const double q = __builtin_nan("");
        va[3 * (size_t)o + 0] = q; va[3 * (size_t)o + 1] = q; va[3 * (size_t)o + 2] = q;
        vh[o] = q;
    }
};
BLOB_KERNEL blob_visc_kernel(BLOB_COMMON, int clip, const int* __restrict__ omap, int n_active,
                             const RecB* __restrict__ recb, const RecBC* __restrict__ bc, const double* __restrict__ m,
                             double* va, double* vh, BlobSel sel, u64* counts) {
    blob_pass(ViscPass{recb, bc, m, va, vh}, n, npad, k, nblk, nbr, slot16, uniq, qorder, clip, omap, n_active, nullptr, sel,
              counts);
}

struct ViscPwPass {
    typedef RecB Rec;
    typedef ViscAcc Sums;
    static constexpr int NSIDE = 1, PER_SLOT = 72;
    static constexpr bool CLIPS = true, VOTES = true, ROW_FROM_LIST = true;
    const RecB* __restrict__ rec;
    const double* __restrict__ rho_s;
    const RecBC* __restrict__ bc;
    const RecSelf* __restrict__ selfr;
    const double* __restrict__ m;
    double *va, *vh;
    struct Row { Q4 r0, rv; double rho_i, cs_i, h_i, mg, hi2, ci, mi; };
    struct Nb { Q8 q; double rho, mc; };
    __device__ __forceinline__ BlobSides sides() const { return {rho_s, 1}; }
    __device__ __forceinline__ Row load_row(int i) const {
        const RecSelf sf = selfr[i];
        const double rho_i = rho_s[i], mci = bc[i].Bw;
        const Q8 s = gload8(&rec[i]);
        return Row{s.lo, s.hi, rho_i, sf.csi, sf.h, sf.mg, s.lo.d, -6.0 * mci, 0.0};
    }
    __device__ __forceinline__ void load_out(Row& r, int o, bool on) const { r.mi = on ? m[o] : 0.0; }
    __device__ __forceinline__ static void row_point(Row& r, const Nb& f) { r.r0 = f.q.lo; r.rv = f.q.hi; }
    __device__ __forceinline__ static bool wanted(const Row&) { return true; }
    __device__ __forceinline__ Nb staged(const double2* img, const double* side, int s, const int* jp) const {
        return Nb{lload8(img, s), side[s], bc[*jp].Bw};
    }
    __device__ __forceinline__ Nb global(int j) const { return Nb{gload8(&rec[j]), rho_s[j], bc[j].Bw}; }
    __device__ __forceinline__ static Nb none(const Row& r) { return Nb{Q8{r.r0, r.rv}, r.rho_i, 0.0}; }
    template <bool CLIP>
    __device__ __forceinline__ double term(Sums& a, const Nb& f, const Row& r) const {
        return visc_pw_term<SqrtMid>(a, f.q.lo, f.q.hi, f.rho, f.mc, r.r0, r.rv, r.rho_i, r.cs_i, r.hi2, r.ci, CLIP);
    }
    __device__ __forceinline__ u64 finish(const Sums& a, double maxrel, const Row& r, int, int o) const {
        va[3 * (size_t)o + 0] = -a.x; va[3 * (size_t)o + 1] = -a.y; va[3 * (size_t)o + 2] = -a.z;
        vh[o] = a.h * r.mi / 2.0;
        return (r.mg > 0.0) ? ct_vote_bits(r.h_i, maxrel) : SPHX_CT_NONE;
    }
};
BLOB_KERNEL blob_visc_pw_kernel(BLOB_COMMON, int clip, const int* __restrict__ omap, int n_active,
                                const RecB* __restrict__ recb, const double* __restrict__ rho_s,
                                const RecBC* __restrict__ bc, const RecSelf* __restrict__ selfr,
                                const double* __restrict__ m, double* va, double* vh, u64* ct_bits, BlobSel sel) {
    blob_pass(ViscPwPass{recb, rho_s, bc, selfr, m, va, vh}, n, npad, k, nblk, nbr, slot16, uniq, qorder, clip, omap, n_active,
              ct_bits, sel);
}

template <int SPEC_MAXM>
__device__ __forceinline__ void species_sweeps(const double (&w)[SPEC_MAXM], double2* img, const u16* tile,
                                               const int* __restrict__ uq, const int* __restrict__ nbr, int n, int npad,
                                               int nm, int p, int i, int t, int half, bool live, int S,
                                               const double* __restrict__ fun, const int* __restrict__ row_of,
                                               const double* __restrict__ m, const AgbTable& agb, int agb_on, double* F,
                                               double* Zout, double* agb_out) {
    double tot[16];
#pragma unroll
    for (int hh = 0; hh < 2; ++hh) {
        __syncthreads();
        {
            int ju[NSTAGE];
#pragma unroll
            for (int r = 0; r < NSTAGE; ++r) {
                const int s = threadIdx.x + r * PASS_T;
                ju[r] = (s < BLOB_S) ? uq[s] : -1;
            }
            double2 c[NSTAGE][4];
#pragma unroll
            for (int r = 0; r < NSTAGE; ++r) {
                const int jr = ju[r] < 0 ? 0 : ju[r];
                const double2* g = reinterpret_cast<const double2*>(fun + (size_t)(row_of ? row_of[jr] : jr) * 16) + 4 * hh;
                c[r][0] = g[0]; c[r][1] = g[1]; c[r][2] = g[2]; c[r][3] = g[3];
            }
#pragma unroll
            for (int r = 0; r < NSTAGE; ++r) {
                const int s = threadIdx.x + r * PASS_T;
                if (ju[r] >= 0) {
                    img[0 * BLOB_S + s] = c[r][0]; img[1 * BLOB_S + s] = c[r][1];
                    img[2 * BLOB_S + s] = c[r][2]; img[3 * BLOB_S + s] = c[r][3];
                }
            }
        }
        __syncthreads();
        double acc[8];
#pragma unroll
        for (int q = 0; q < 8; ++q) acc[q] = 0.0;
#pragma unroll
        for (int mm = 0; mm < SPEC_MAXM; ++mm) {
            if (mm < nm) {
                const unsigned sl = tile[(LPP * mm + half) * BLOB_P + t];
                if (sl != SLOT_NONE && live) {
                    Q4 f0, f1;
                    if (sl < SLOT_OVER) { f0 = lload4(img, (int)sl, 0); f1 = lload4(img, (int)sl, 1); }
                    else {
                        const int jo = nbr[(size_t)(LPP * mm + half) * npad + p];
                        const double* q = fun + (size_t)(row_of ? row_of[jo] : jo) * 16 + 8 * hh;
                        f0 = gload4(q); f1 = gload4(q + 4);
                    }
                    const double wm = w[mm];
                    acc[0] += wm * f0.a; acc[1] += wm * f0.b; acc[2] += wm * f0.c; acc[3] += wm * f0.d;
                    acc[4] += wm * f1.a; acc[5] += wm * f1.b; acc[6] += wm * f1.c; acc[7] += wm * f1.d;
                }
            }
        }
#pragma unroll
        for (int q = 0; q < 8; ++q) tot[8 * hh + q] = group_total(acc[q]);
    }
    if (live && !half) {
#pragma unroll
        for (int q = 0; q < 16; ++q)
            if (q < S) F[(size_t)q * n + i] = tot[q];
    }
    if (live && agb_on) {
        const double Z = species_metallicity(agb, tot, S);
        if (!half) Zout[i] = Z;
        const double Mi = m[i];
        double* row = agb_out + (size_t)i * S;
        for (int q = half; q < S; q += LPP)
            if (!((agb.covered >> q) & 1u)) row[q] = 0.0;
        for (int o = half; o < agb.nspl; o += LPP) {
            double val;
            const int target = agb_one_spline(agb, o, Mi, Z, val);
            if (target >= 0) row[target] = val;
        }
    }
}

template <int SPEC_MAXM>
__global__ __launch_bounds__(PASS_T, PASS_MINW) void blob_density_species_kernel(int n, int npad, int k, int nblk,
        const int* __restrict__ nbr, const u16* __restrict__ slot16, const int* __restrict__ uniq,
        const int* __restrict__ qorder, int clip, const RecA* __restrict__ rec, double* rho_s, double* rho, double* rhod,
        double* nden, double* G, double* ha,
        int S, const double* __restrict__ fun, const int* __restrict__ row_of, const double* __restrict__ m, AgbTable agb,
        int agb_on, double* F, double* Zout, double* agb_out) {
    const DensityPass ps{rec, rho_s, rho, rhod, nden, G, ha};
    double2* img = BlobLds<0>::img();
    u16* tile = BlobLds<0>::tile();
    const int t = threadIdx.x / LPP, half = threadIdx.x & (LPP - 1);
    const int nm = KPAD(k) / LPP;
    for (int bi = blockIdx.x; bi < nblk; bi += gridDim.x) {
        const int b = xcd_block(bi, nblk);
        const int p = b * BLOB_P + t;
        const bool live = p < n;
        const int i = live ? qorder[p] : 0;
        const int* uq = uniq + (size_t)b * BLOB_S;
        stage<0>(img, nullptr, tile, rec, nullptr, 0, nullptr, 0, uq, slot16, npad, k, b);
        DensityPass::Row row = ps.load_row(i);
        __syncthreads();
        double w[SPEC_MAXM];
#pragma unroll
        for (int mm = 0; mm < SPEC_MAXM; ++mm) w[mm] = 0.0;
        if (live) {
            blob_row_point(ps, row, nbr, p, t);
// ... 70 lines not shown
        }
        species_sweeps(w, img, tile, uq, nbr, n, npad, nm, p, i, t, half, live, S, fun, row_of, m, agb, agb_on, F, Zout, agb_out);
        __syncthreads();
    }
}

#define DRAG_XLDS (BLOB_S * (2 * sizeof(int) + 1))
template <bool FILL>
__global__ __launch_bounds__(PASS_T, PASS_MINW) void blob_drag_kernel(int n, int npad, int k, int nblk,
                                                           const int* __restrict__ nbr,
                                                           const u16* __restrict__ slot16,
                                                           const int* __restrict__ uniq,
                                                           const int* __restrict__ qorder,
                                                           const RecB* __restrict__ recb,
                                                           const double* __restrict__ m,
                                                           const double* __restrict__ ptype,
                                                           const double* __restrict__ mgm,
                                                           const double* __restrict__ mcs,
                                                           const int* __restrict__ id, double* onto, DragScatter sc) {
    extern __shared__ double2 img[];
    u16* tile = reinterpret_cast<u16*>(img + (FILL ? 4 * BLOB_S : 0));
    int* cntL = reinterpret_cast<int*>(tile + KPAD(k) * BLOB_P);
    int* baseL = cntL + BLOB_S;
    unsigned char* dust = reinterpret_cast<unsigned char*>(baseL + BLOB_S);
    const int t = threadIdx.x / LPP, part = threadIdx.x & (LPP - 1);
    const int nm = KPAD(k) / LPP;
    for (int bi = blockIdx.x; bi < nblk; bi += gridDim.x) {
        const int b = xcd_block(bi, nblk);
        const int p = b * BLOB_P + t;
        const bool live = p < n;
        const int i = live ? qorder[p] : 0;
        const int* uq = uniq + (size_t)b * BLOB_S;
        if (FILL) {
            stage<0>(img, nullptr, tile, recb, nullptr, 0, nullptr, 0, uq, slot16, npad, k, b);
        } else {
            const int pieces = KPAD(k) * (BLOB_P / 8);
            for (int q = threadIdx.x; q < pieces; q += PASS_T) {
                const int kk = q / (BLOB_P / 8), c = q % (BLOB_P / 8);
                uint4 v = make_uint4(0xFFFFFFFFu, 0xFFFFFFFFu, 0xFFFFFFFFu, 0xFFFFFFFFu);
                if (kk < k) v = *reinterpret_cast<const uint4*>(slot16 + (size_t)kk * npad + (size_t)b * BLOB_P + c * 8);
                *reinterpret_cast<uint4*>(tile + kk * BLOB_P + c * 8) = v;
            }
        }
        for (int s = threadIdx.x; s < BLOB_S; s += PASS_T) {
            const int j = uq[s];
            dust[s] = (j >= 0 && ptype[j] == 2.0) ? 1 : 0;
            cntL[s] = 0;
        }
        __syncthreads();
        if (live) {
            for (int m0 = 0; m0 < nm; ++m0) {
                const int kk = LPP * m0 + part;
                const unsigned sl = tile[kk * BLOB_P + t];
                if (sl < SLOT_OVER) {
                    if (dust[sl] && uq[sl] != i) atomicAdd(&cntL[sl], 1);
                } else if (sl == SLOT_OVER && !FILL) {
                    const int j = nbr[(size_t)kk * npad + p];
                    if (j != i && ptype[j] == 2.0) atomicAdd(&sc.cnt[j], 1);
                }
            }
        }
        __syncthreads();
        if (!FILL) {
            for (int s = threadIdx.x; s < BLOB_S; s += PASS_T)
                if (cntL[s]) atomicAdd(&sc.cnt[uq[s]], cntL[s]);
            __syncthreads();
            continue;
        }
        for (int s = threadIdx.x; s < BLOB_S; s += PASS_T) {
            const int c = cntL[s];
            if (c) {
                const int j = uq[s];
                baseL[s] = sc.start[j] + atomicSub(&sc.cnt[j], c) - c;
                cntL[s] = 0;
            }
        }
        const double* rq = reinterpret_cast<const double*>(&recb[i]);
        const Q4 r0 = gload4(rq), rv = gload4(rq + 4);
        __syncthreads();
        double ox = 0.0, oy = 0.0, oz = 0.0;
        if (live) {
            unsigned dm = 0;
            for (int m0 = 0; m0 < nm; ++m0) {
                const int kk = LPP * m0 + part;
                const unsigned sl = tile[kk * BLOB_P + t];
                bool d = false;
                if (sl < SLOT_OVER) d = dust[sl] != 0;
                else if (sl == SLOT_OVER) d = ptype[nbr[(size_t)kk * npad + p]] == 2.0;
                dm |= (d ? 1u : 0u) << m0;
            }
            while (dm) {
                const int m0 = __builtin_ctz(dm);
                dm &= dm - 1;
                const int kk = LPP * m0 + part;
                const unsigned sl = tile[kk * BLOB_P + t];
                int j;
                Q4 q0, qv;
                if (sl < SLOT_OVER) {
                    j = uq[sl];
                    q0 = lload4(img, (int)sl, 0); qv = lload4(img, (int)sl, 1);
                } else {
                    j = nbr[(size_t)kk * npad + p];
                    const double* qb = reinterpret_cast<const double*>(&recb[j]);
                    q0 = gload4(qb); qv = gload4(qb + 4);
                }
                const Vec3 f = drag_term(ox, oy, oz, q0, qv, r0, rv, j, m, mgm, mcs);
                if (j != i) {
                    const int slot = (sl < SLOT_OVER) ? baseL[sl] + atomicAdd(&cntL[sl], 1)
                                                      : sc.start[j] + atomicSub(&sc.cnt[j], 1) - 1;
                    sphx_drag_put(sc, slot, ((u64)(unsigned)id[i] << 8) | (u64)kk, -f.x, -f.y, -f.z);
                }
            }
        }
        const double tx = group_total(ox), ty = group_total(oy), tz = group_total(oz);
        if (live && part == 0) { onto[3 * (size_t)i] = tx; onto[3 * (size_t)i + 1] = ty; onto[3 * (size_t)i + 2] = tz; }
        __syncthreads();
    }
}

BlobSel sphx_blob_sel(sphx_ctx* ctx, int part) {
    if (!ctx->blob_split_valid) return BlobSel{nullptr, nullptr, 0};
    const int* list = ctx->blob_split.as<int>();
    return BlobSel{list, list + (size_t)ctx->blob_split_nblk, part == 0 ? 3 : part};
}

int sphx_blob_grid(sphx_ctx* ctx, int nblk) {
    if (ctx->blob_grid <= 0) {
        int cus = 256;
        (void)hipDeviceGetAttribute(&cus, hipDeviceAttributeMultiprocessorCount, ctx->device);
        ctx->blob_grid = ((cus * 2 + 7) / 8) * 8;
    }
    return nblk < ctx->blob_grid ? nblk : ctx->blob_grid;
}

int sphx_lds_opt_in(sphx_ctx* ctx, const void* kernel, size_t bytes) {
    for (int q = 0; q < ctx->n_lds_raised; ++q)
        if (ctx->lds_raised[q] == kernel) return SPHX_OK;
    if (ctx->n_lds_raised == SPHX_LDS_KERNELS)
        return sphx_set_err(ctx, SPHX_E_HIP, "sphx_lds_opt_in: more than %d kernels", SPHX_LDS_KERNELS);
    HIPCHK(hipFuncSetAttribute(kernel, hipFuncAttributeMaxDynamicSharedMemorySize, (int)bytes));
    ctx->lds_raised[ctx->n_lds_raised++] = kernel;
    return SPHX_OK;
}

static int blob_n_active(const sphx_ctx* ctx, int64_t n) { return ctx->map_perm ? ctx->map_nactive : (int)n; }

int sphx_blob_density(sphx_ctx* ctx, int64_t n, int k, bool lean) {
    return blob_launch(ctx, blob_density_kernel, DensityPass::PER_SLOT, 0, n, k, ctx->clip_grad, ctx->map_perm,
                       blob_n_active(ctx, n), ctx->rec1.as<RecA>(), ctx->rho_s.as<double>(), ctx->rho.as<double>(),
                       ctx->rhod.as<double>(), ctx->nden.as<double>(), lean ? nullptr : ctx->G.as<double>(), ctx->ha.as<double>(),
                       sphx_blob_sel(ctx, ctx->pass_part));
}

int sphx_blob_pi(sphx_ctx* ctx, int64_t n, int k, u64* ct_bits) {
    return blob_launch(ctx, blob_pi_kernel, PiPass::PER_SLOT, 0, n, k, ctx->map_perm, blob_n_active(ctx, n), ctx->recv.as<RecB>(),
                       ctx->rho_s.as<double>(), ctx->self_s.as<RecSelf>(), ctx->bc_s.as<RecBC>(), ctx->Pi.as<double>(),
                       ctx->map_perm ? ctx->Bw.as<double>() : nullptr, ct_bits, sphx_blob_sel(ctx, ctx->pass_part),
                       ctx->scal.as<u64>() + SC_SETTLED);
}

int sphx_blob_visc(sphx_ctx* ctx, int64_t n, int k, const double* m) {
    return blob_launch(ctx, blob_visc_kernel, ViscPass::PER_SLOT, 0, n, k, ctx->clip_grad, ctx->map_perm, blob_n_active(ctx, n),
                       ctx->recv.as<RecB>(), ctx->bc_s.as<RecBC>(), m, ctx->va.as<double>(), ctx->vh.as<double>(),
                       sphx_blob_sel(ctx, ctx->pass_part), ctx->scal.as<u64>() + SC_SETTLED);
}

int sphx_blob_visc_pw(sphx_ctx* ctx, int64_t n, int k, const double* m, u64* ct_bits) {
    return blob_launch(ctx, blob_visc_pw_kernel, ViscPwPass::PER_SLOT, 0, n, k, ctx->clip_grad, ctx->map_perm,
                       blob_n_active(ctx, n), ctx->recv.as<RecB>(), ctx->rho_s.as<double>(), ctx->bc_s.as<RecBC>(),
                       ctx->self_s.as<RecSelf>(), m, ctx->va.as<double>(), ctx->vh.as<double>(), ct_bits, sphx_blob_sel(ctx, ctx->pass_part));
}

int sphx_blob_density_species(sphx_ctx* ctx, int64_t n, int k, bool lean, int S, const double* fun, const int* row_of,
                              const double* m_sorted, double* F, double* Z, double* agb, int agb_on) {
    const auto kern = (KPAD(k) / LPP <= 10) ? blob_density_species_kernel<10> : blob_density_species_kernel<16>;
    return blob_launch(ctx, kern, 64, 0, n, k, ctx->clip_grad, ctx->rec1.as<RecA>(), ctx->rho_s.as<double>(), ctx->rho.as<double>(),
                       ctx->rhod.as<double>(), ctx->nden.as<double>(), lean ? nullptr : ctx->G.as<double>(),
                       ctx->ha.as<double>(), S, fun, row_of, m_sorted, ctx->agb, agb_on, F, Z, agb);
}

int sphx_blob_species(sphx_ctx* ctx, int64_t n, int k, int S, const double* fun, const int* row_of, const double* m_sorted, double* F,
                      double* Z, double* agb, int agb_on) {
    const auto kern = (KPAD(k) / LPP <= 10) ? blob_species_kernel<10> : blob_species_kernel<16>;
    return blob_launch(ctx, kern, 64, 0, n, k, S, ctx->rec1.as<RecA>(), fun, row_of, m_sorted, ctx->agb, agb_on, F, Z, agb);
}

int sphx_blob_drag(sphx_ctx* ctx, int64_t n, int k, bool count_only, const double* m, const double* ptype, const double* mgm,
                   const double* mcs, const int* id, double* onto, const DragScatter& sc) {
    if (count_only)
        return blob_launch(ctx, blob_drag_kernel<false>, 0, DRAG_XLDS, n, k, nullptr, m, ptype, mgm, mcs, id, onto, sc);
    return blob_launch(ctx, blob_drag_kernel<true>, 64, DRAG_XLDS, n, k, ctx->recv.as<RecB>(), m, ptype, mgm, mcs, id, onto, sc);
}
```

### sph-code_amd/csrc/sphx_internal.h

```cpp
#pragma once
#include <hip/hip_runtime.h>
#include <stdint.h>
#include <stdio.h>
#include <string.h>
#include <math.h>
#include <float.h>
#include <vector>
#include "../../include/sphx.h"
#include "sphx_agb.h"

#define SPHX_WAVE 64
#define SPHX_W6_C 1.5666814710608448

typedef unsigned long long u64;
typedef unsigned int u32;
struct PinnedLayout;

struct DevBuf {
    void* p = nullptr;
    size_t cap = 0;
    template <class T> T* as() const { return (T*)p; }
};

struct __attribute__((aligned(64))) RecA {
// ... 111 lines not shown
struct sphx_ctx {
    int device = 0;
    hipStream_t stream = nullptr;
    hipStream_t own_stream = nullptr;
    hipStream_t side_stream = nullptr;
    sphx_constants cst;
    char tunables[1024] = {0};
    double rscale = 1.08, cell_factor = 0.55;
    double rscale_build = 1.3;
    bool use_verlet = false;
    bool use_blob = true;
    int blob_curve = 0;
    bool use_group = true;
    bool use_lds = true;
    bool drag_lds = true;
    bool blob_split_on = true;
    bool species_lds = true;
    bool species_fused = true;
    int blob_grid = 0;
    int blob_slots = 1 << 20;
    int olev_mode = 2;
    int distrust_mode = 0;
    bool cell_feedback = true;
    double cell_fb_hi = 0.30, cell_fb_lo = 0.10;
    int64_t max_cells = 0;
    double box_sigmas = 3.0;
    double h_clip_factor = 8.0;
    double reach_cap = 0.0;
    bool timing_detail = false;
    int clip_grad = 0;
    int visc_mode = 0;
    bool drag = false;
    int loop_forms = 0;
    double loop_d = 0.0;
    int gravity = 0;
    double grav_G = 0.0;
    int grav_order = 2;
    bool grav_per_thread = false;
    int grav_ws = 1;
    bool agb_on = false;
    AgbTable agb;
    double dev_hmean = 0.0;

    char err[512] = {0};
    sphx_stats stats;
    int64_t n = 0, npad = 0;
    int k = 0, s = 0;
    int sp = 0;
    bool has_state = false;
    int64_t step_count = 0;
    double dt_last = 0.0;
    bool tprev_valid = false;
    bool ct_primed = false;
    bool recs_pw = false;
    bool nbr_api_valid = false;
    int64_t nbr_api_n = 0;
    int nbr_api_k = 0;
    bool step_list_valid = false;
    const int* step_qorder = nullptr;
    int64_t step_list_n = 0;
    int step_list_k = 0;
    bool list_valid = false;
    int64_t list_n = 0;
    int list_k = 0;
    const int* map_perm = nullptr;
    int map_nactive = 0;
    const int* qorder = nullptr;
    bool blob_lists = false;
    bool blob_split_valid = false;
    int blob_split_nblk = 0;
    int pass_part = 0;
    bool loop2_interior_done = false;
    bool dev_ev_pending = false;
    const double *dev_drag_on = nullptr, *dev_drag_re = nullptr, *dev_drag_rho = nullptr, *dev_drag_rhod = nullptr;
    const double* dev_grav = nullptr;
    bool gx_built = false;
    int64_t gx_n = 0, gx_nowned = 0;
    Pyr gx_py;
    GravRef gx_ref;
    GridParams grid;
    const double* tbox = nullptr;
    double tbox_h[6] = {0, 0, 0, 0, 0, 0};
    double clip_lo[3] = {0, 0, 0}, clip_hi[3] = {0, 0, 0};
    bool clip_valid = false;
    double h_clip = 0.0;
    double cell_scale = 1.0;
    bool cells_unsorted = false;
    bool curve_counted = false;
    bool order_by_count = false;
    bool blob_scatter_pending = false;
    BlobBits blob_scatter_bits;
    const int* blob_scatter_mstart = nullptr;
    bool bbox_ticket_zeroed = false;
    const void* cell_fill_zeroed = nullptr;
    const void* mcount_zeroed = nullptr;
    int mcount_zeroed_M = 0;
    const void* fcount_zeroed = nullptr;
    int64_t fcount_zeroed_n = 0;
    const void* tie_list_cleared = nullptr;
    const int* tie_count_dev = nullptr;
    int tie_cap_last = 0;
    const void* ds_cnt_zeroed = nullptr;
    const void* olev_fill_zeroed = nullptr;
    unsigned lbs_epoch[2] = {0u, 0u};
    const void* lds_raised[SPHX_LDS_KERNELS] = {nullptr};
    int n_lds_raised = 0;
    OutLevels olev;
    bool olev_ev_valid = false;
    u64 farq_seen = 0;
    int64_t farq_last = 0;
    int64_t list_len_last = 0;
    bool knn_lag_valid = false;
    u64 knn_lag[10] = {0, 0, 0, 0, 0, 0, 0, 0, 0, 0};
    u64 densep_seen = 0;
    int64_t densep_last = 0;
    u64 crowded_seen = 0;
    int64_t crowded_last = 0;
    bool distrust = false;
    u64 badhint_seen = 0;
    bool ev_detail[3] = {false, false, false};
    int ev_has07[3] = {0, 0, 0};
    unsigned ev_pending = 0;
    hipEvent_t lag_balias[2] = {nullptr, nullptr}, lag_halias[2] = {nullptr, nullptr};
    bool lag_bvalid[2] = {false, false}, lag_hvalid[2] = {false, false};
    int64_t lag_bn[2] = {0, 0};
    int lag_bslot = 0, lag_hslot = 0;

    std::vector<void*> allocs;
    DevBuf rec1, recv;
    DevBuf rho_s, bc_s, self_s;
    DevBuf drag_on, drag_re;
    DevBuf need_pyr;
    DevBuf fun_id;
    DevBuf crowded;
    DevBuf loop_side;
    DevBuf ds_cnt, ds_start, ds_ent;
    DevBuf lrec_a, lrec_v;
    DevBuf grav, grav_sort, grav_tmp;
    DevBuf grav_pyr, grav_cell;
    DevBuf grav_quad;
    DevBuf gx_pts, gx_m, gx_ord, gx_map, gx_box, gx_cflag, gx_coff, gx_pcnt, gx_poff, gx_counts;
    DevBuf list64, dref, pos0, pos4;
    DevBuf nbr;
    DevBuf porder, mcount, mstart;
    DevBuf agb_knots, Zmet, agb_dust;
    DevBuf fail_list;
    DevBuf olev_start, olev_fill, olev_list, olev_key;
    DevBuf lbs_state[2];
    DevBuf cell_rank;
    DevBuf perm_fin;
    DevBuf tie_list;
    DevBuf slot16, uniq;
    DevBuf blob_class, blob_split;
    DevBuf rho, rhod, nden, G, Pi, Bw, va, vh, ha, F;
    DevBuf scal;
    DevBuf cell_of, cell_start, cell_fill, perm, inv, scan_tmp, bbox_tmp;
    DevBuf in_a, in_b, in_c, in_d, in_e, in_f, in_g, in_h, in_i, in_j, out_a, out_b, out_c;
    DevBuf idx64, dist_out, nontriv, h_api;
    DevBuf arb_rec, arb_wrec, arb_flag, arb_cmax, arb_q, arb_key, arb_tmp, arb_acc, arb_out, arb_red;
    DevBuf arb_pos, arb_cs, arb_perm;
    int64_t arb_ball_id = 0, arb_ball_n = 0, arb_ball_m = 0;
    GridParams arb_g;
    double arb_tb[6] = {0, 0, 0, 0, 0, 0};
    StageTimer arb_t;
    DevBuf rad_in, rad_soa, rad_ray, rad_part, rad_gas, rad_out;
    StageTimer rad_t;
    DevBuf cool_in, cool_nb, cool_rec, cool_int, cool_rev, cool_tab, cool_out, cool_tmp;
    StageTimer cool_t;
    DevBuf dust_in, dust_nb, dust_rec, dust_int, dust_rev, dust_out, dust_tmp;
    double dust_kn[40] = {0};
    StageTimer dust_t;
    DevBuf chem_in, chem_nb, chem_rec, chem_int, chem_row, chem_rowi, chem_rev, chem_first, chem_out, chem_tmp;
    double chem_tab[4 * SPHX_MAX_SPECIES] = {0};
    StageTimer chem_t{5};
    DevBuf phase_int, phase_out;
    double phase_tab[4 * SPHX_MAX_SPECIES] = {0};
    StageTimer phase_t{5};
    StateArrays st, alt;
    DevBuf badc;
    DevBuf scal_tmp;
    DevBuf hsum_tmp;
    hipEvent_t ev_join = nullptr;
    hipEvent_t ev_perm = nullptr;
    hipEvent_t olev_ev = nullptr;
    hipEvent_t ev[10] = {nullptr};
    hipEvent_t evring[3][10] = {{nullptr}};
    hipEvent_t lag_bev[2] = {nullptr, nullptr}, lag_hev[2] = {nullptr, nullptr};
    PinnedLayout* pinned = nullptr;
};

int sphx_set_err(sphx_ctx* ctx, int code, const char* fmt, ...);
int sphx_ensure(sphx_ctx* ctx, DevBuf& b, size_t bytes, hipStream_t in_use_on);
static inline int sphx_ensure(sphx_ctx* ctx, DevBuf& b, size_t bytes) { return sphx_ensure(ctx, b, bytes, ctx->stream); }
void sphx_release(sphx_ctx* ctx, DevBuf& b);

#define HIPCHK(expr)                                                                         \
    do {                                                                                     \
        hipError_t e_ = (expr);                                                              \
        if (e_ != hipSuccess)                                                                \
            return sphx_set_err(ctx, SPHX_E_HIP, "%s:%d %s -> %s", __FILE__, __LINE__,       \
                                #expr, hipGetErrorString(e_));                               \
    } while (0)
#define NEED(p)                                                                              \
    do {                                                                                     \
        if (!(p)) return sphx_set_err(ctx, SPHX_E_ARG, "%s: argument %s is NULL", __func__, #p); \
    } while (0)
#define SPHX_TRY(expr)                                                                       \
    do {                                                                                     \
        int r_ = (expr);                                                                     \
        if (r_ != SPHX_OK) return r_;                                                        \
    } while (0)

static inline void sphx_step_list_drop(sphx_ctx* ctx) { ctx->step_list_valid = false; ctx->step_qorder = nullptr; }
static inline int64_t sphx_pad64(int64_t n) { return (n + 63) & ~int64_t(63); }

__device__ __forceinline__ int xcd_block(int b, int nb) {
    const int q = nb >> 3, r = nb & 7, x = b & 7, s = b >> 3;
    return x * q + (x < r ? x : r) + s;
}

#ifndef SPHX_SUM_PARTS
#define SPHX_SUM_PARTS 4
#endif

__device__ __forceinline__ double sphx_nan_to_num(double v) {
    if (v != v) return 0.0;
    if (v > DBL_MAX) return DBL_MAX;
    if (v < -DBL_MAX) return -DBL_MAX;
    return v;
}

#define SPHX_CT_NONE 0x7FF0000000000000ull
int sphx_prime_ct(sphx_ctx* ctx, u64* ct_bits);

enum {
    SC_CT_BITS = 0,
    SC_DT = 1,
    SC_CAND = 2,
    SC_RETRY = 3,
    SC_HSUM = 4,
    SC_DISP2 = 5,
    SC_NFAIL = 6,
    SC_HCNT = 7,
    SC_GRAV_EPS = 8,
    SC_NFAILQ = 9,
    SC_SHORT = 10,
    SC_FARQ = 11,
    SC_BADHINT = 12,
    SC_CROWDED = 13,
    SC_DENSEP = 14,
    SC_KGDBG = 16,
    SC_SETTLED = 24,
    SC_NSLOTS = 26
};

enum {
    BAD_ACCEL = 0,
    BAD_ENERGY = 1,
    BAD_STATE = 2,
    BAD_H = 3,
    BADC_BUCKETS = 64, BADC_STRIDE = 16
};
int sphx_badc_read(sphx_ctx* ctx);

struct PinnedSide { double red[4]; int count; int pad_[7]; u64 cand; };
struct PinnedLag {
    double box[32];
    double hs[32];
};
struct PinnedLayout {
    union {
        u64 scal[SC_NSLOTS];
        PinnedSide side;
    };
    char pad0_[256 - SC_NSLOTS * 8];
    double hsum[4];
    char pad1_[1024 - 256 - 4 * 8];
    PinnedLag lag[2];
    char pad2_[3072 - 1024 - 2 * 512];
    u64 knn_lag[10];
    char pad3_[8192 - 3072 - 10 * 8];
    u64 badc[BADC_BUCKETS * BADC_STRIDE];
};
static_assert(sizeof(PinnedLayout) == 16384, "ctx->pinned is 16 KiB");
static_assert(offsetof(PinnedLayout, side) == 0 && offsetof(PinnedSide, count) == 32 && offsetof(PinnedSide, cand) == 64 &&
                  offsetof(PinnedLayout, hsum) == 256 && offsetof(PinnedLayout, lag) == 1024 && sizeof(PinnedLag) == 512 &&
                  offsetof(PinnedLag, hs) == 256 && offsetof(PinnedLayout, knn_lag) == 3072 && offsetof(PinnedLayout, badc) == 8192,
              "the offsets in use since the members were byte counts");
#define SPHX_PIN_APART(a, b) \
    static_assert(offsetof(PinnedLayout, a) + sizeof(PinnedLayout::a) <= offsetof(PinnedLayout, b), #a " overlaps " #b)
SPHX_PIN_APART(scal, hsum); SPHX_PIN_APART(side, hsum); SPHX_PIN_APART(hsum, lag); SPHX_PIN_APART(lag, knn_lag);
SPHX_PIN_APART(knn_lag, badc);
#undef SPHX_PIN_APART
static_assert(offsetof(PinnedLayout, badc) + sizeof(PinnedLayout::badc) == sizeof(PinnedLayout), "the buckets end the block");

struct CopyF64 { const void* host; const void* dev; size_t count; };
int sphx_upload_f64(sphx_ctx* ctx, const CopyF64* t, int nt);
int sphx_download_f64(sphx_ctx* ctx, const CopyF64* t, int nt);

int sphx_bbox(sphx_ctx* ctx, int64_t n, const double* x, const double* y, const double* z,
              double out_minmax[13], bool use_clip);
int sphx_median(sphx_ctx* ctx, int64_t n, const double* v, double* out_dev);
int sphx_gravity_launch(sphx_ctx* ctx, int64_t n, const double* x, const double* y, const double* z, int ps,
                        const double* m, const double* eps_dev, double eps, double G, const int* omap,
                        double* acc);
int sphx_gravity_tree_launch(sphx_ctx* ctx, int64_t n, const double* x, const double* y, const double* z,
                             const double* m, int ws, const double* eps_dev, double eps, double G, const int* omap,
                             double* acc);
int sphx_dev_collect(sphx_ctx* ctx);
int sphx_loop_step_sums(sphx_ctx* ctx, int64_t n, int k, double d);
int sphx_build_blob_order(sphx_ctx* ctx, int64_t n, bool defer_scatter = false);
static inline double sphx_cell_feedback(sphx_ctx* ctx, int64_t n) {
    if (ctx->cell_feedback && n > 0) {
        const double dense = (double)ctx->densep_last / (double)n;
        if (dense > ctx->cell_fb_hi) ctx->cell_scale = ctx->cell_scale * 0.97 > 0.35 ? ctx->cell_scale * 0.97 : 0.35;
        else if (dense < ctx->cell_fb_lo) ctx->cell_scale = ctx->cell_scale * 1.01 < 1.0 ? ctx->cell_scale * 1.01 : 1.0;
    }
    return ctx->cell_scale;
}
int sphx_blob_translate(sphx_ctx* ctx, int64_t n, int k);
int sphx_blob_density_species(sphx_ctx* ctx, int64_t n, int k, bool lean, int S, const double* fun, const int* row_of,
                              const double* m_sorted, double* F, double* Z, double* agb, int agb_on);
int sphx_blob_density(sphx_ctx* ctx, int64_t n, int k, bool lean);
int sphx_blob_pi(sphx_ctx* ctx, int64_t n, int k, u64* ct_bits);
int sphx_blob_visc(sphx_ctx* ctx, int64_t n, int k, const double* m);
int sphx_blob_visc_pw(sphx_ctx* ctx, int64_t n, int k, const double* m, u64* ct_bits);
int sphx_blob_species(sphx_ctx* ctx, int64_t n, int k, int S, const double* fun, const int* row_of, const double* m_sorted, double* F,
                      double* Z, double* agb, int agb_on);
#define CELL_SORT_SERIAL 16
#define CELL_SORT_WAVE 512
int sphx_cell_cues(sphx_ctx* ctx, hipStream_t stream);
struct OrderFinish {
    int n;
    GridParams g; BlobBits b;
    const int *perm_in, *cell_of, *cell_start, *mstart;
    int *perm_out, *porder, *mcount;
};
int sphx_finish_order_only(sphx_ctx* ctx, const OrderFinish& o);
struct GridBuildOpts {
    bool lagged = false;
    hipEvent_t alias_ev = nullptr;
    bool sort_cells_later = false;
    bool count_curve = false;
    double* clamp_vel[3] = {nullptr, nullptr, nullptr};
};
int sphx_build_grid(sphx_ctx* ctx, int64_t n, int k, const double* x, const double* y, const double* z, double cell_hint,
                    const GridBuildOpts& opts = GridBuildOpts());
struct GridHostState {
    GridParams grid;
    const double* tbox;
    double tbox_h[6], clip_lo[3], clip_hi[3], cell_size;
    bool clip_valid, cells_unsorted;
    int olev_L;
    int64_t cells;
    const int *map_perm, *qorder;
};
GridHostState sphx_grid_host_save(const sphx_ctx* ctx);
void sphx_grid_host_restore(sphx_ctx* ctx, const GridHostState& saved);
int sphx_excl_scan_int(sphx_ctx* ctx, const int* in, int* out, int n);
struct alignas(32) DragEntry { u64 key; double x, y, z; };
struct DragScatter { int* cnt; const int* start; DragEntry* ent; };
__device__ __forceinline__ void sphx_drag_put(const DragScatter& sc, int slot, u64 key, double x, double y, double z) {
    double2* q = reinterpret_cast<double2*>(sc.ent + slot);
    q[0] = make_double2(__longlong_as_double((long long)key), x);
    q[1] = make_double2(y, z);
}
int sphx_drag_scatter_plan(sphx_ctx* ctx, int64_t n, int k, const int* nbr, const double* ptype, const int* qorder, DragScatter* out,
                           bool blob = false);
int sphx_drag_scatter_reduce(sphx_ctx* ctx, int64_t n, const DragScatter& d, double* react);
int sphx_blob_drag(sphx_ctx* ctx, int64_t n, int k, bool count_only, const double* m, const double* ptype, const double* mgm,
                   const double* mcs, const int* id, double* onto, const DragScatter& sc);
int sphx_build_outlier_levels(sphx_ctx* ctx, int64_t n, const double* xs, const double* ys, const double* zs);
struct KnnIn {
    const double *xs, *ys, *zs;
    const int32_t* id;
    const int32_t* inv = nullptr;
    const double* rsearch = nullptr;
    double rscale = 1.0, rbound = 0.0;
    bool hinted = false;
    bool hint_by_id = false;
    bool lag_external = false;
};
struct KnnOut {
    int32_t* nbr;
    int32_t* list64 = nullptr;
    double* dref = nullptr;
    double* h_sorted;
    int64_t* idx64;
    double* dist;
    int64_t* nontriv;
    double* h_by_id;
};
int sphx_knn(sphx_ctx* ctx, int64_t n, int k, const KnnIn& in, const KnnOut& out);
struct PrepIn {
    const double *x, *y, *z; int ps;
    const double *vx, *vy, *vz; int vs;
    const double *m, *h, *T, *mu, *gam, *ptype;
    void pos_aos(const double* p) { x = p; y = p + 1; z = p + 2; ps = 3; }
    void vel_aos(const double* v) { vx = v; vy = v + 1; vz = v + 2; vs = 3; }
};
int sphx_prep(sphx_ctx* ctx, int64_t n, const PrepIn& in, bool pairwise, hipStream_t stream);
int sphx_pass_density(sphx_ctx* ctx, int64_t n, int k, bool lean = false);
int sphx_pass_pi(sphx_ctx* ctx, int64_t n, int k, const double* h, const double* ptype);
int sphx_pass_visc(sphx_ctx* ctx, int64_t n, int k, const double* m);
int sphx_pass_visc_pw(sphx_ctx* ctx, int64_t n, int k, const double* m);
int sphx_pass_species(sphx_ctx* ctx, int64_t n, int k, int s, const double* fun, double* F);
int sphx_step_species(sphx_ctx* ctx, int64_t n, int k);
int sphx_species_on(sphx_ctx* ctx, int64_t n, int k, int S, int SP, const double* fun, const int* row_of, const double* m_sorted,
                    double* F, double* Z, double* agb);
int sphx_agb_table_set(sphx_ctx* ctx, int S, int nspl, const int32_t* ntx, const int32_t* nty, const double* tx, const double* ty,
                       const double* coeffs, const int32_t* mapto, double divisor, const double* mu_specie, double solar_mass);
int sphx_transpose_nbr(sphx_ctx* ctx, int64_t n, int k, const int64_t* nb_rowmajor);

int sphx_loop_density_dev(sphx_ctx* ctx, int64_t n, int k, const int* nbr, const double* points, const double* mass,
                          const double* ptype, double d, double m_0, double* out);
struct ChemDev { double *pos, *m, *mu, *sizes, *T, *ptype, *fun, *tab; };
struct ChemPar { double d, dt, k_B, m_0, symax; };
struct ChemRes { double *mass_new, *fun_new; unsigned long long* counters; unsigned long long hc[8]; size_t M; int64_t rounds; };
int sphx_chem_check_shape(sphx_ctx* ctx, const char* who, int64_t n, int k, int s);
int sphx_chem_check_scalars(sphx_ctx* ctx, const char* who, double d, double dt, const double mrn[2], double k_B, double amu, double m_0);
int sphx_chem_tables(sphx_ctx* ctx, const char* who, int s, const double* mu_specie, const double* mineral_densities,
                     const double* sputtering_yields, const double mrn[2], double amu, double* symax_out);
int sphx_chem_ints(sphx_ctx* ctx, int64_t n, int k, int** nbr);
int sphx_chem_inputs(sphx_ctx* ctx, int64_t n, int s, ChemDev* in);
int sphx_chem_run(sphx_ctx* ctx, const char* who, int64_t n, int k, int s, const ChemDev& in, const int* nbr, const ChemPar& par,
                  StageTimer* t, ChemRes* res);
void sphx_chem_counts(sphx_ctx* ctx, ChemRes* res, int64_t* counts);
struct DustDev { double *pos, *vel, *m, *mu, *sizes, *dens, *ptype, *fun; };
struct DustPar { double crit_mass, crit_density, amu; unsigned sel, si; int fraction; };
struct DustRes { double *destr, *reup; unsigned long long* counters; };
int sphx_dust_check_shape(sphx_ctx* ctx, const char* who, int64_t n, int k, int s);
int sphx_dust_check_scalars(sphx_ctx* ctx, const char* who, double crit_mass, double critical_density, int guard_mode);
int sphx_dust_params(sphx_ctx* ctx, const char* who, int s, double crit_mass, double critical_density, const int32_t* species_curve,
                     const double knots_v[8], const double knots_c[8], const double knots_si[8], int guard_mode, DustPar* par);
int sphx_dust_inputs(sphx_ctx* ctx, int64_t n, int s, DustDev* in);
int sphx_dust_run(sphx_ctx* ctx, const char* who, int64_t n, int k, int s, const DustDev& in, const int* nbr_given, const DustPar& par,
                  StageTimer* t, DustRes* res);

int sphx_clamp(sphx_ctx* ctx, int64_t n, StateArrays& s);
int sphx_permute_state(sphx_ctx* ctx, int64_t n, bool split, hipEvent_t after_first);
int sphx_hsum(sphx_ctx* ctx, int64_t n, const double* h, hipStream_t stream);
int sphx_compute_dt(sphx_ctx* ctx, int first, double fixed_dt);
int sphx_integrate(sphx_ctx* ctx, int64_t n, int fold_dt = 0, int first = 0, double fixed_dt = 0.0);
int sphx_pass_drag(sphx_ctx* ctx, int64_t n, int k, const double* m, const double* ptype, const double* mgm,
                   const double* mcs);
int sphx_aos_to_soa3(sphx_ctx* ctx, int64_t n, const double* aos, double* x, double* y, double* z);
int sphx_soa3_to_aos_by_id(sphx_ctx* ctx, int64_t n, const int* id, const double* x, const double* y,
                           const double* z, double* aos);
int sphx_scatter_rows_by_id(sphx_ctx* ctx, int64_t n, int w, const int* id, const double* in, double* out);
int sphx_gather3(sphx_ctx* ctx, int64_t n, const int* perm, const double* x, const double* y,
                 const double* z, double* xs, double* ys, double* zs);
int sphx_iota(sphx_ctx* ctx, int64_t n, int* out);
int sphx_knn_refresh(sphx_ctx* ctx, int64_t n, int k, const double* x, const double* y, const double* z,
                     int32_t* nbr, double* h_sorted, int64_t* nfail_out);
int sphx_save_list_positions(sphx_ctx* ctx, int64_t n, const double* x, const double* y, const double* z);
```

### sph-code_amd/csrc/sphx_sums.hip

```cpp
#include "sphx_internal.h"
#include "sphx_wave.h"
#include "sphx_pair.h"
#pragma clang fp contract(off)
#include <float.h>
#include <stdlib.h>

struct PrepArgs {
    int n;
    const double *x, *y, *z; int ps;
    const double *vx, *vy, *vz; int vs;
    const double *m, *h, *T, *mu, *gam, *ptype;
    double kB, amu;
    RecA* ra; RecB* rb; RecBC* bc; RecSelf* self;
    const int* perm;
    int which, n_active;
    int pairwise;
};

__global__ __launch_bounds__(256) void prep_kernel(PrepArgs a) {
    const int t = blockIdx.x * blockDim.x + threadIdx.x;
    if (t >= a.n) return;
    const int i = a.perm ? a.perm[t] : t;
    if (a.which && ((i < a.n_active) != (a.which == 1))) return;
    const double m = a.m[i], h = a.h[i], T = a.T[i], mu = a.mu[i], gam = a.gam[i], pt = a.ptype[i];
// ... 33 lines not shown
    a.m = in.m; a.h = in.h; a.T = in.T; a.mu = in.mu; a.gam = in.gam; a.ptype = in.ptype;
    a.kB = ctx->cst.k_B; a.amu = ctx->cst.amu;
    a.ra = ctx->rec1.as<RecA>();
    a.rb = ctx->recv.as<RecB>();
    a.bc = ctx->bc_s.as<RecBC>();
    a.self = ctx->self_s.as<RecSelf>();
    a.perm = ctx->map_perm;
    a.which = ctx->map_perm ? ctx->pass_part : 0;
    a.n_active = ctx->map_nactive;
    a.pairwise = pairwise ? 1 : 0;
    ctx->recs_pw = pairwise;
    hipLaunchKernelGGL(prep_kernel, dim3((unsigned)((n + 255) / 256)), dim3(256), 0, stream, a);
    HIPCHK(hipGetLastError());
    return SPHX_OK;
}

__global__ __launch_bounds__(256) void transpose_nbr_kernel(long long n, int k, int npad,
                                                            const long long* nb, int* out) {
    long long e = (long long)blockIdx.x * blockDim.x + threadIdx.x;
    if (e >= n * k) return;
    long long i = e / k;
    int kk = (int)(e - i * k);
    long long j = nb[e];
    out[(long long)kk * npad + i] = (j >= 0 && j < n) ? (int)j : -1;
}

int sphx_transpose_nbr(sphx_ctx* ctx, int64_t n, int k, const int64_t* nb_dev) {
    int64_t npad = sphx_pad64(n);
    sphx_step_list_drop(ctx);
    SPHX_TRY(sphx_ensure(ctx, ctx->nbr, (size_t)k * npad * sizeof(int)));
    HIPCHK(hipMemsetAsync(ctx->nbr.p, 0xFF, (size_t)k * npad * sizeof(int), ctx->stream));
    long long tot = (long long)n * k;
    hipLaunchKernelGGL(transpose_nbr_kernel, dim3((unsigned)((tot + 255) / 256)), dim3(256), 0,
                       ctx->stream, (long long)n, k, (int)npad, (const long long*)nb_dev,
                       ctx->nbr.as<int>());
    HIPCHK(hipGetLastError());
    return SPHX_OK;
}

struct OutMap { const int* perm; int n_active; };
__device__ __forceinline__ int out_index(const OutMap& m, int i) { return m.perm ? m.perm[i] : i; }

#define NBATCH 4

__global__ __launch_bounds__(256) void pass_density_kernel(int n, int npad, int k, int clip,
                                                           const int* __restrict__ nbr,
                                                           const RecA* __restrict__ rec, double* rho_s,
                                                           const int* __restrict__ qorder, OutMap om, double* rho,
                                                           double* rhod, double* nden, double* G,
                                                           double* ha) {
    const int p = xcd_block(blockIdx.x, gridDim.x) * blockDim.x + threadIdx.x;
    if (p >= n) return;
    const int i = qorder ? qorder[p] : p;
    const int o = out_index(om, i);
    if (o >= om.n_active) return;
    const double* self = reinterpret_cast<const double*>(&rec[i]);
    const Q4 s0 = gload4(self), s1 = gload4(self + 4);
    int j0 = nbr[p];
    double xr = s0.a, yr = s0.b, zr = s0.c;
    if (j0 >= 0 && j0 != i) { xr = rec[j0].x; yr = rec[j0].y; zr = rec[j0].z; }
    const double hi2 = s0.d, ci = -6.0 * s1.a, Ai = s1.c;
    DensAcc acc[SPHX_SUM_PARTS] = {};
    for (int kk0 = 0; kk0 < k; kk0 += NBATCH) {
      int jb[NBATCH];
      Q4 q0b[NBATCH], q1b[NBATCH];
#pragma unroll
      for (int u = 0; u < NBATCH; ++u) jb[u] = (kk0 + u < k) ? nbr[(size_t)(kk0 + u) * npad + p] : -1;
#pragma unroll
      for (int u = 0; u < NBATCH; ++u) {
          const double* q = reinterpret_cast<const double*>(&rec[jb[u] < 0 ? i : jb[u]]);
          q0b[u] = gload4(q); q1b[u] = gload4(q + 4);
      }
#pragma unroll
      for (int u = 0; u < NBATCH; ++u) {
        if (jb[u] < 0) continue;
        density_term<SqrtLib>(acc[u & (SPHX_SUM_PARTS - 1)], q0b[u], q1b[u], xr, yr, zr, hi2, ci, Ai, clip != 0);
      }
    }
    const double s_rho = parts_total(acc, &DensAcc::rho), s_rd = parts_total(acc, &DensAcc::rd), s_n = parts_total(acc, &DensAcc::n);
    const double gx = parts_total(acc, &DensAcc::gx), gy = parts_total(acc, &DensAcc::gy), gz = parts_total(acc, &DensAcc::gz);
    rho[o] = s_rho; rhod[o] = s_rd; nden[o] = s_n;
    rho_s[i] = s_rho;
    if (G) { G[3 * (size_t)o + 0] = -gx; G[3 * (size_t)o + 1] = -gy; G[3 * (size_t)o + 2] = -gz; }
    ha[3 * (size_t)o + 0] = -gx / s_rho;
    ha[3 * (size_t)o + 1] = -gy / s_rho;
    ha[3 * (size_t)o + 2] = -gz / s_rho;
}

int sphx_pass_density(sphx_ctx* ctx, int64_t n, int k, bool lean) {
    SPHX_TRY(sphx_ensure(ctx, ctx->rho, (size_t)n * sizeof(double)));
    SPHX_TRY(sphx_ensure(ctx, ctx->rhod, (size_t)n * sizeof(double)));
    SPHX_TRY(sphx_ensure(ctx, ctx->nden, (size_t)n * sizeof(double)));
    SPHX_TRY(sphx_ensure(ctx, ctx->G, (size_t)n * 3 * sizeof(double)));
    SPHX_TRY(sphx_ensure(ctx, ctx->ha, (size_t)n * 3 * sizeof(double)));
    if (ctx->qorder && ctx->blob_lists) return sphx_blob_density(ctx, n, k, lean);
    hipLaunchKernelGGL(pass_density_kernel, dim3((unsigned)((n + 255) / 256)), dim3(256), 0, ctx->stream,
                       (int)n, (int)sphx_pad64(n), k, ctx->clip_grad, ctx->nbr.as<int>(), ctx->rec1.as<RecA>(),
                       ctx->rho_s.as<double>(), ctx->qorder, OutMap{ctx->map_perm, ctx->map_perm ? ctx->map_nactive : (int)n},
                       ctx->rho.as<double>(), ctx->rhod.as<double>(), ctx->nden.as<double>(),
                       lean ? nullptr : ctx->G.as<double>(), ctx->ha.as<double>());
    HIPCHK(hipGetLastError());
    return SPHX_OK;
}

__global__ __launch_bounds__(256) void pass_pi_kernel(int n, int npad, int k, const int* __restrict__ nbr,
                                                      const RecB* __restrict__ recb,
                                                      const double* __restrict__ rho_s,
                                                      const RecSelf* __restrict__ selfr, RecBC* bc,
                                                      const int* __restrict__ qorder, OutMap om, double* Pi, double* BwOut,
                                                      u64* ct_bits) {
    const int p = xcd_block(blockIdx.x, gridDim.x) * blockDim.x + threadIdx.x;
    u64 my_ct = SPHX_CT_NONE;
    const int i = (p < n) ? (qorder ? qorder[p] : p) : n;
    const int o = (i < n) ? out_index(om, i) : 0x7FFFFFFF;
    if (i < n && o < om.n_active) {
        int j0 = nbr[p];
        if (j0 < 0) j0 = i;
        const double* rq = reinterpret_cast<const double*>(&recb[j0]);
        const Q4 r0 = gload4(rq), rv = gload4(rq + 4);
        const RecSelf sf = selfr[i];
        const double rho_i = rho_s[i], cs_i = sf.csi, ms_i = sf.mg, h_i = sf.h;
        double a_pi[SPHX_SUM_PARTS] = {}, maxrel = 0.0;
        for (int kk0 = 0; kk0 < k; kk0 += NBATCH) {
          int jb[NBATCH];
          Q4 q0b[NBATCH], qvb[NBATCH];
          double rhob[NBATCH];
#pragma unroll
          for (int u = 0; u < NBATCH; ++u) jb[u] = (kk0 + u < k) ? nbr[(size_t)(kk0 + u) * npad + p] : -1;
#pragma unroll
          for (int u = 0; u < NBATCH; ++u) {
              const int jj = jb[u] < 0 ? i : jb[u];
              const double* qb = reinterpret_cast<const double*>(&recb[jj]);
              q0b[u] = gload4(qb); qvb[u] = gload4(qb + 4);
              rhob[u] = rho_s[jj];
          }
#pragma unroll
          for (int u = 0; u < NBATCH; ++u) {
            if (jb[u] < 0) continue;
            const PiPair t = pi_term<SqrtLib>(q0b[u], qvb[u], rhob[u], r0, rv, rho_i, cs_i);
            a_pi[u & (SPHX_SUM_PARTS - 1)] += t.pi;
            maxrel = fmax(maxrel, t.rel);
          }
        }
        const double s_pi = parts_total(a_pi);
        Pi[o] = s_pi;
        const double bw = fmax(ms_i, 0.0) * s_pi;
        bc[i].Bw = bw;
        if (BwOut) BwOut[o] = bw;
        if (ms_i > 0.0) my_ct = ct_vote_bits(h_i, maxrel);
    }
    block_min_vote<256>(my_ct, ct_bits);
}

int sphx_pass_pi(sphx_ctx* ctx, int64_t n, int k, const double* h, const double* ptype) {
    (void)ptype; (void)h;
    SPHX_TRY(sphx_ensure(ctx, ctx->Pi, (size_t)n * sizeof(double)));
    SPHX_TRY(sphx_ensure(ctx, ctx->Bw, (size_t)n * sizeof(double)));
    u64* ct = ctx->scal.as<u64>() + SC_CT_BITS;
    if (!ctx->ct_primed) SPHX_TRY(sphx_prime_ct(ctx, ct));
    ctx->ct_primed = false;
    if (ctx->qorder && ctx->blob_lists) return sphx_blob_pi(ctx, n, k, ct);
    hipLaunchKernelGGL(pass_pi_kernel, dim3((unsigned)((n + 255) / 256)), dim3(256), 0, ctx->stream,
                       (int)n, (int)sphx_pad64(n), k, ctx->nbr.as<int>(), ctx->recv.as<RecB>(),
                       ctx->rho_s.as<double>(), ctx->self_s.as<RecSelf>(), ctx->bc_s.as<RecBC>(), ctx->qorder,
                       OutMap{ctx->map_perm, ctx->map_perm ? ctx->map_nactive : (int)n},
                       ctx->Pi.as<double>(), ctx->map_perm ? ctx->Bw.as<double>() : nullptr, ct);
    HIPCHK(hipGetLastError());
    return SPHX_OK;
}

__global__ __launch_bounds__(256) void pass_visc_kernel(int n, int npad, int k, int clip,
                                                        const int* __restrict__ nbr,
                                                        const RecB* __restrict__ recb,
                                                        const RecBC* __restrict__ bc,
                                                        const int* __restrict__ qorder, OutMap om,
                                                        const double* __restrict__ m, double* va,
                                                        double* vh) {
    const int p = xcd_block(blockIdx.x, gridDim.x) * blockDim.x + threadIdx.x;
    if (p >= n) return;
    const int i = qorder ? qorder[p] : p;
    const int o = out_index(om, i);
    if (o >= om.n_active) return;
    int j0 = nbr[p];
    if (j0 < 0) j0 = i;
    const double* rq = reinterpret_cast<const double*>(&recb[j0]);
    const Q4 r0 = gload4(rq), rv = gload4(rq + 4);
    const double2 bci = *reinterpret_cast<const double2*>(&bc[i]);
    const double hi2 = recb[i].h2, ci = -6.0 * bci.y, Bi = bci.x;
    ViscAcc acc[SPHX_SUM_PARTS] = {};
    for (int kk0 = 0; kk0 < k; kk0 += NBATCH) {
      int jb[NBATCH];
      Q4 q0b[NBATCH], qvb[NBATCH];
      double2 bcb[NBATCH];
#pragma unroll
      for (int u = 0; u < NBATCH; ++u) jb[u] = (kk0 + u < k) ? nbr[(size_t)(kk0 + u) * npad + p] : -1;
#pragma unroll
      for (int u = 0; u < NBATCH; ++u) {
          const int jj = jb[u] < 0 ? i : jb[u];
          const double* qb = reinterpret_cast<const double*>(&recb[jj]);
          q0b[u] = gload4(qb); qvb[u] = gload4(qb + 4);
          bcb[u] = *reinterpret_cast<const double2*>(&bc[jj]);
      }
#pragma unroll
      for (int u = 0; u < NBATCH; ++u) {
        if (jb[u] < 0) continue;
        visc_term<SqrtLib>(acc[u & (SPHX_SUM_PARTS - 1)], q0b[u], qvb[u], bcb[u].x, bcb[u].y, r0, rv, hi2, ci, Bi, clip != 0);
      }
    }
    const double ax = parts_total(acc, &ViscAcc::x), ay = parts_total(acc, &ViscAcc::y), az = parts_total(acc, &ViscAcc::z);
    const double heat = parts_total(acc, &ViscAcc::h);
    va[3 * (size_t)o + 0] = -ax; va[3 * (size_t)o + 1] = -ay; va[3 * (size_t)o + 2] = -az;
    vh[o] = heat * m[o] / 2.0;
}

int sphx_pass_visc(sphx_ctx* ctx, int64_t n, int k, const double* m) {
    SPHX_TRY(sphx_ensure(ctx, ctx->va, (size_t)n * 3 * sizeof(double)));
    SPHX_TRY(sphx_ensure(ctx, ctx->vh, (size_t)n * sizeof(double)));
    if (ctx->qorder && ctx->blob_lists) return sphx_blob_visc(ctx, n, k, m);
    hipLaunchKernelGGL(pass_visc_kernel, dim3((unsigned)((n + 255) / 256)), dim3(256), 0, ctx->stream,
                       (int)n, (int)sphx_pad64(n), k, ctx->clip_grad, ctx->nbr.as<int>(), ctx->recv.as<RecB>(),
                       ctx->bc_s.as<RecBC>(), ctx->qorder,
                       OutMap{ctx->map_perm, ctx->map_perm ? ctx->map_nactive : (int)n}, m,
                       ctx->va.as<double>(), ctx->vh.as<double>());
    HIPCHK(hipGetLastError());
    return SPHX_OK;
}

__global__ __launch_bounds__(256) void pass_visc_pw_kernel(int n, int npad, int k, int clip,
                                                           const int* __restrict__ nbr,
                                                           const RecB* __restrict__ recb,
                                                           const double* __restrict__ rho_s,
                                                           const RecBC* __restrict__ bc,
                                                           const RecSelf* __restrict__ selfr,
                                                           const int* __restrict__ qorder, OutMap om,
                                                           const double* __restrict__ m, double* va, double* vh,
                                                           u64* ct_bits) {
    const int p = xcd_block(blockIdx.x, gridDim.x) * blockDim.x + threadIdx.x;
    u64 my_ct = SPHX_CT_NONE;
    const int i = (p < n) ? (qorder ? qorder[p] : p) : n;
    const int o = (i < n) ? out_index(om, i) : 0x7FFFFFFF;
    if (i < n && o < om.n_active) {
        int j0 = nbr[p];
        if (j0 < 0) j0 = i;
        const double* rq = reinterpret_cast<const double*>(&recb[j0]);
        const Q4 r0 = gload4(rq), rv = gload4(rq + 4);
        const RecSelf sf = selfr[i];
        const double rho_i = rho_s[i], cs_i = sf.csi, h_i = sf.h;
        const double hi2 = recb[i].h2, ci = -6.0 * bc[i].Bw;
        ViscAcc acc[SPHX_SUM_PARTS] = {};
        double maxrel = 0.0;
        for (int kk0 = 0; kk0 < k; kk0 += NBATCH) {
          int jb[NBATCH];
          Q4 q0b[NBATCH], qvb[NBATCH];
          double rhob[NBATCH], mcb[NBATCH];
#pragma unroll
          for (int u = 0; u < NBATCH; ++u) jb[u] = (kk0 + u < k) ? nbr[(size_t)(kk0 + u) * npad + p] : -1;
#pragma unroll
          for (int u = 0; u < NBATCH; ++u) {
              const int jj = jb[u] < 0 ? i : jb[u];
              const double* qb = reinterpret_cast<const double*>(&recb[jj]);
              q0b[u] = gload4(qb); qvb[u] = gload4(qb + 4);
              rhob[u] = rho_s[jj];
              mcb[u] = bc[jj].Bw;
          }
#pragma unroll
          for (int u = 0; u < NBATCH; ++u) {
            if (jb[u] < 0) continue;
            maxrel = fmax(maxrel, visc_pw_term<SqrtLib>(acc[u & (SPHX_SUM_PARTS - 1)], q0b[u], qvb[u], rhob[u], mcb[u], r0, rv,
                                                         rho_i, cs_i, hi2, ci, clip != 0));
          }
        }
        const double ax = parts_total(acc, &ViscAcc::x), ay = parts_total(acc, &ViscAcc::y), az = parts_total(acc, &ViscAcc::z);
        const double heat = parts_total(acc, &ViscAcc::h);
        va[3 * (size_t)o + 0] = -ax; va[3 * (size_t)o + 1] = -ay; va[3 * (size_t)o + 2] = -az;
        vh[o] = heat * m[o] / 2.0;
        if (sf.mg > 0.0) my_ct = ct_vote_bits(h_i, maxrel);
    }
    block_min_vote<256>(my_ct, ct_bits);
}

int sphx_pass_visc_pw(sphx_ctx* ctx, int64_t n, int k, const double* m) {
    SPHX_TRY(sphx_ensure(ctx, ctx->va, (size_t)n * 3 * sizeof(double)));
    SPHX_TRY(sphx_ensure(ctx, ctx->vh, (size_t)n * sizeof(double)));
    u64* ct = ctx->scal.as<u64>() + SC_CT_BITS;
    if (!ctx->ct_primed) SPHX_TRY(sphx_prime_ct(ctx, ct));
    ctx->ct_primed = false;
    if (ctx->qorder && ctx->blob_lists) return sphx_blob_visc_pw(ctx, n, k, m, ct);
    hipLaunchKernelGGL(pass_visc_pw_kernel, dim3((unsigned)((n + 255) / 256)), dim3(256), 0, ctx->stream,
                       (int)n, (int)sphx_pad64(n), k, ctx->clip_grad, ctx->nbr.as<int>(), ctx->recv.as<RecB>(),
                       ctx->rho_s.as<double>(), ctx->bc_s.as<RecBC>(), ctx->self_s.as<RecSelf>(), ctx->qorder,
                       OutMap{ctx->map_perm, ctx->map_perm ? ctx->map_nactive : (int)n}, m,
                       ctx->va.as<double>(), ctx->vh.as<double>(), ct);
    HIPCHK(hipGetLastError());
    return SPHX_OK;
}

__global__ __launch_bounds__(256) void drag_count_kernel(int n, int npad, int k, const int* __restrict__ nbr,
                                                         const double* __restrict__ ptype, const int* __restrict__ qorder,
                                                         int* cnt) {
    const int p = blockIdx.x * blockDim.x + threadIdx.x;
    if (p >= n) return;
    const int i = qorder ? qorder[p] : p;
    for (int kk = 0; kk < k; ++kk) {
        const int j = nbr[(size_t)kk * npad + p];
        if (j >= 0 && j != i && ptype[j] == 2.0) atomicAdd(&cnt[j], 1);
    }
}
#define DRAG_RED_BLOCKS 2048
#define DRAG_RED_U 4
template <int U>
__device__ __forceinline__ void drag_slice_sum(int s, int L, const DragEntry* __restrict__ ent,
                                               double* pk, int lane, double& acc) {
    u64 key[U];
    double vx[U], vy[U], vz[U];
    int rank[U];
#pragma unroll
    for (int u = 0; u < U; ++u) {
        const int q = lane + 64 * u;
        key[u] = ~0ull; vx[u] = vy[u] = vz[u] = 0.0;
        if (q < L) {
            const double2* e = reinterpret_cast<const double2*>(ent + s + q);
            const double2 e0 = e[0], e1 = e[1];
            key[u] = (u64)__double_as_longlong(e0.x); vx[u] = e0.y; vy[u] = e1.x; vz[u] = e1.y;
        }
        rank[u] = 0;
    }
#pragma unroll
    for (int c = 0; c < U; ++c) {
        const int lc = L - 64 * c < 64 ? L - 64 * c : 64;
        for (int t = 0; t < lc; ++t) {
            const u64 kt = ((u64)(unsigned)__builtin_amdgcn_readlane((int)(key[c] >> 32), t) << 32) |
                           (u64)(unsigned)__builtin_amdgcn_readlane((int)key[c], t);
#pragma unroll
            for (int u = 0; u < U; ++u) rank[u] += kt < key[u] ? 1 : 0;
        }
    }
#pragma unroll
    for (int u = 0; u < U; ++u) {
        const int q = lane + 64 * u;
        if (q < L) { pk[3 * rank[u]] = vx[u]; pk[3 * rank[u] + 1] = vy[u]; pk[3 * rank[u] + 2] = vz[u]; }
    }
    wave_sync();
    if (lane < 3) {
        int t = 0;
        for (; t + 8 <= L; t += 8) {
            double v[8];
#pragma unroll
            for (int q = 0; q < 8; ++q) v[q] = pk[3 * (t + q) + lane];
#pragma unroll
            for (int q = 0; q < 8; ++q) acc += v[q];
        }
        for (; t < L; ++t) acc += pk[3 * t + lane];
    }
    wave_sync();
}
__global__ __launch_bounds__(256) void drag_reduce_kernel(int n, const int* __restrict__ start,
                                                          const DragEntry* __restrict__ ent, double* react) {
    __shared__ double parked[4][64 * DRAG_RED_U * 3];
    const int lane = threadIdx.x & 63, wave = threadIdx.x >> 6;
    double* pk = parked[wave];
    for (int j0 = (blockIdx.x * 4 + wave) * 64; j0 < n; j0 += gridDim.x * 4 * 64) {
        const int jl = j0 + lane;
        int sl = 0, Ll = 0;
        if (jl < n) { sl = start[jl]; Ll = start[jl + 1] - sl; }
        if (jl < n && Ll == 0) { react[3 * (size_t)jl] = 0.0; react[3 * (size_t)jl + 1] = 0.0; react[3 * (size_t)jl + 2] = 0.0; }
        u64 todo = __builtin_amdgcn_ballot_w64(Ll > 0);
        while (todo) {
            const int t = __builtin_ctzll(todo);
            todo &= todo - 1;
            const int s = __builtin_amdgcn_readlane(sl, t), L = __builtin_amdgcn_readlane(Ll, t);
            const int j = j0 + t;
// ... 230 lines not shown
```

Baseline: 942.1 million.

## Mark settled blobs in Pi pass and compact viscosity work to live blobs

```diff
diff --git a/include/sphx.h b/include/sphx.h
--- a/include/sphx.h
+++ b/include/sphx.h
@@ -64,6 +64,7 @@
     int64_t tie_capacity;
     int64_t visc_blobs_settled;
     int64_t pi_waves_settled;
+    int64_t visc_launches_skipped;
 } sphx_stats;
 
 int         sphx_create(sphx_ctx** out, int device);
diff --git a/sph-code_amd/_lib.py b/sph-code_amd/_lib.py
--- a/sph-code_amd/_lib.py
+++ b/sph-code_amd/_lib.py
@@ -27,7 +27,8 @@
                 ("ms_species", C.c_double), ("short_rows", C.c_int64), ("detail_steps", C.c_int64), ("far_queries", C.c_int64),
                 ("outlier_levels", C.c_int64), ("bad_accel", C.c_int64), ("bad_energy", C.c_int64), ("bad_state", C.c_int64),
                 ("bad_h", C.c_int64), ("search_steps", C.c_int64), ("tie_entries", C.c_int64), ("tie_capacity", C.c_int64),
-                ("visc_blobs_settled", C.c_int64), ("pi_waves_settled", C.c_int64)]
+                ("visc_blobs_settled", C.c_int64), ("pi_waves_settled", C.c_int64),
+                ("visc_launches_skipped", C.c_int64)]
 
     def as_dict(self):
         return {n: getattr(self, n) for n, _ in self._fields_}
diff --git a/sph-code_amd/csrc/sphx_api.hip b/sph-code_amd/csrc/sphx_api.hip
--- a/sph-code_amd/csrc/sphx_api.hip
+++ b/sph-code_amd/csrc/sphx_api.hip
@@ -671,9 +671,15 @@
         if (ctx->visc_mode == 1) {
             SPHX_TRY(sphx_pass_visc_pw(ctx, n, k, s.m.as<double>()));
         } else {
-            SPHX_TRY(sphx_pass_pi(ctx, n, k, s.hprev.as<double>(), s.ptype.as<double>()));
+            const bool hand_visc = sphx_blob_can_hand_visc(ctx, n);
+            if (hand_visc) {
+                SPHX_TRY(sphx_ensure(ctx, ctx->va, (size_t)n * 3 * sizeof(double)));
+                SPHX_TRY(sphx_ensure(ctx, ctx->vh, (size_t)n * sizeof(double)));
+                SPHX_TRY(sphx_blob_size_marks(ctx, n));
+            }
+            SPHX_TRY(sphx_pass_pi(ctx, n, k, s.hprev.as<double>(), s.ptype.as<double>(), hand_visc));
             if (detail) HIPCHK(hipEventRecord(ev[5], ctx->stream));
-            SPHX_TRY(sphx_pass_visc(ctx, n, k, s.m.as<double>()));
+            SPHX_TRY(sphx_pass_visc(ctx, n, k, s.m.as<double>(), hand_visc));
         }
     }
     if (ctx->drag)
@@ -968,12 +974,13 @@
         if (ctx->map_perm) ctx->stats.fallback_queries = (int64_t)(u32)nfail;
     }
     if (ctx->scal.p) {
-        u64 cnt[2] = {0, 0};
+        u64 cnt[3] = {0, 0, 0};
         HIPCHK(hipSetDevice(ctx->device));
         HIPCHK(hipMemcpyAsync(cnt, ctx->scal.as<u64>() + SC_SETTLED, sizeof(cnt), hipMemcpyDeviceToHost, ctx->stream));
         HIPCHK(hipStreamSynchronize(ctx->stream));
         ctx->stats.visc_blobs_settled = (int64_t)cnt[0];
         ctx->stats.pi_waves_settled = (int64_t)cnt[1];
+        ctx->stats.visc_launches_skipped = (int64_t)cnt[2];
     }
     *out = ctx->stats;
     for (int w = 0; w < 2; ++w) {
@@ -997,7 +1004,7 @@
     memset(&ctx->stats, 0, sizeof(ctx->stats));
     HIPCHK(hipMemsetAsync(ctx->scal.as<u64>() + SC_CAND, 0, 2 * sizeof(u64), ctx->stream));
     HIPCHK(hipMemsetAsync(ctx->scal.as<u64>() + SC_SHORT, 0, sizeof(u64), ctx->stream));
-    HIPCHK(hipMemsetAsync(ctx->scal.as<u64>() + SC_SETTLED, 0, 2 * sizeof(u64), ctx->stream));
+    HIPCHK(hipMemsetAsync(ctx->scal.as<u64>() + SC_SETTLED, 0, 3 * sizeof(u64), ctx->stream));
     HIPCHK(hipMemsetAsync(ctx->badc.p, 0, (size_t)BADC_BUCKETS * BADC_STRIDE * sizeof(u64), ctx->stream));
     HIPCHK(hipStreamSynchronize(ctx->stream));
     return SPHX_OK;
diff --git a/sph-code_amd/csrc/sphx_blob.h b/sph-code_amd/csrc/sphx_blob.h
--- a/sph-code_amd/csrc/sphx_blob.h
+++ b/sph-code_amd/csrc/sphx_blob.h
@@ -181,7 +181,9 @@
 template <class P> struct BlobSettles<P, decltype((void)P::SETTLES)> { static constexpr bool value = P::SETTLES; };
 template <class P, class = void> struct BlobSaturates { static constexpr bool value = false; };
 template <class P> struct BlobSaturates<P, decltype((void)P::SATURATES)> { static constexpr bool value = P::SATURATES; };
-enum { BLOB_CNT_BLOBS_SETTLED = 0, BLOB_CNT_WAVES_SATURATED = 1 };
+template <class P, class = void> struct BlobHandsOn { static constexpr bool value = false; };
+template <class P> struct BlobHandsOn<P, decltype((void)P::HANDS_ON)> { static constexpr bool value = P::HANDS_ON; };
+enum { BLOB_CNT_BLOBS_SETTLED = 0, BLOB_CNT_WAVES_SATURATED = 1, BLOB_CNT_LAUNCHES_SKIPPED = 2 };
 struct BlobSides { const double* g0 = nullptr; int s0 = 0; const double* g1 = nullptr; int s1 = 0; };
 
 template <int NSIDE>
@@ -277,6 +279,15 @@
         if (r) atomicAdd(dst, (u64)r);
     }
 }
+#define BLOB_OWN_MAX 64
+__device__ __forceinline__ int* blob_own_list() {
+    __shared__ int own[BLOB_OWN_MAX];
+    return own;
+}
+__device__ __forceinline__ int* blob_live_flag() {
+    __shared__ int flag;
+    return &flag;
+}
 template <class P>
 __device__ __forceinline__ void blob_row_point(const P& ps, typename P::Row& row, const int* __restrict__ nbr, int p,
                                                int t) {
@@ -290,19 +301,27 @@
 __device__ __forceinline__ void blob_pass(const P& ps, int n, int npad, int k, int nblk, const int* __restrict__ nbr,
                                           const u16* __restrict__ slot16, const int* __restrict__ uniq,
                                           const int* __restrict__ qorder, int clip, const int* __restrict__ omap,
-                                          int n_active, u64* ct_bits, const BlobSel& sel, u64* counts = nullptr) {
+                                          int n_active, u64* ct_bits, const BlobSel& sel, u64* counts = nullptr,
+                                          int own_n = -1) {
     static_assert(P::PER_SLOT == 64 + (P::NSIDE ? 8 : 0), "image bytes per slot: the record and one side value");
-    constexpr bool SETTLES = BlobSettles<P>::value, SATURATES = BlobSaturates<P>::value;
+    constexpr bool SETTLES = BlobSettles<P>::value, SATURATES = BlobSaturates<P>::value, HANDS_ON = BlobHandsOn<P>::value;
     static_assert(!SATURATES || LPP == 4, "sphx_wave_saturated: a row's lanes are one nibble of the wave's mask");
     typedef BlobLds<P::NSIDE> L;
     const BlobSides sd = ps.sides();
     const int t = threadIdx.x / LPP, half = threadIdx.x & (LPP - 1);
     u64 my_ct = SPHX_CT_NONE;
     unsigned blobs_settled = 0, waves_saturated = 0;
-    const int nsel = blob_sel_count(sel, nblk);
+    if constexpr (HANDS_ON) {
+        if (threadIdx.x == 0) *blob_live_flag() = 0;
+    }
     const int stride = gridDim.x;
+    const bool own = own_n >= 0;
+    const int nsel = own ? (own_n ? (int)blockIdx.x + (own_n - 1) * stride + 1 : 0) : blob_sel_count(sel, nblk);
+    auto blob_at = [&](int bq) -> int {
+        return own ? blob_own_list()[(bq - (int)blockIdx.x) / stride] : blob_sel_at(sel, bq, nsel);
+    };
     auto particle_of = [&](int bq) -> int {
-        const int pq = blob_sel_at(sel, bq, nsel) * BLOB_P + t;
+        const int pq = blob_at(bq) * BLOB_P + t;
         return (pq < n) ? qorder[pq] : 0;
     };
     auto nothing_left = [&](const RowAhead& r) -> bool {
@@ -314,19 +333,19 @@
     unsigned round = 0;
     if constexpr (SETTLES) {
         if ((int)blockIdx.x < nsel)
-            cur = blob_row_ahead(ps, particle_of(blockIdx.x), blob_sel_at(sel, blockIdx.x, nsel) * BLOB_P + t, n, slot16, omap);
+            cur = blob_row_ahead(ps, particle_of(blockIdx.x), blob_at(blockIdx.x) * BLOB_P + t, n, slot16, omap);
         if ((int)blockIdx.x + stride < nsel) i_next = particle_of(blockIdx.x + stride);
         blob_settled = block_all_at_barrier<PASS_T>(nothing_left(cur), round++);
     }
     for (int bi = blockIdx.x; bi < nsel; bi += stride) {
-        const int b = blob_sel_at(sel, bi, nsel);
+        const int b = blob_at(bi);
         const int p = b * BLOB_P + t;
         int i, o;
         bool settled = false;
         auto fetch_ahead = [&]() {
             if constexpr (SETTLES) {
                 if (bi + stride < nsel) {
-                    cur = blob_row_ahead(ps, i_next, blob_sel_at(sel, bi + stride, nsel) * BLOB_P + t, n, slot16, omap);
+                    cur = blob_row_ahead(ps, i_next, blob_at(bi + stride) * BLOB_P + t, n, slot16, omap);
                     if (bi + 2 * stride < nsel) i_next = particle_of(bi + 2 * stride);
                 }
             }
@@ -393,13 +412,23 @@
                 group_total_fields(a);
                 if (P::VOTES) mx = group_max(mx);
                 if (!half) {
-                    const u64 cb = ps.finish(a, mx, row, i, o);
+                    u64 cb;
+                    if constexpr (HANDS_ON) {
+                        bool live = false;
+                        cb = ps.finish(a, mx, row, i, o, L::tile()[t] != SLOT_NONE, live);
+                        if (live) *blob_live_flag() = 1;
+                    } else {
+                        cb = ps.finish(a, mx, row, i, o);
+                    }
                     my_ct = cb < my_ct ? cb : my_ct;
                 }
             }
         }
         if constexpr (SETTLES) blob_settled = block_all_at_barrier<PASS_T>(nothing_left(cur), round++);
         else __syncthreads();
+        if constexpr (HANDS_ON) {
+            if (ps.hands_on() && threadIdx.x == 0) { ps.hand_on(b, *blob_live_flag() != 0); *blob_live_flag() = 0; }
+        }
     }
     if (P::VOTES) block_min_vote<PASS_T>(my_ct, ct_bits);
     if constexpr (SETTLES) {
diff --git a/sph-code_amd/csrc/sphx_blob.hip b/sph-code_amd/csrc/sphx_blob.hip
--- a/sph-code_amd/csrc/sphx_blob.hip
+++ b/sph-code_amd/csrc/sphx_blob.hip
@@ -237,17 +237,28 @@
               n_active, nullptr, sel);
 }
 
+__device__ __forceinline__ void visc_settle_store(double* va, double* vh, int o) {
+    const double q = __builtin_nan("");
+    va[3 * (size_t)o + 0] = q; va[3 * (size_t)o + 1] = q; va[3 * (size_t)o + 2] = q;
+    vh[o] = q;
+}
+
 struct PiPass {
     typedef RecB Rec;
     struct Sums { double pi; };
     static constexpr int NSIDE = 1, PER_SLOT = 72;
     static constexpr bool CLIPS = false, VOTES = true, ROW_FROM_LIST = true;
     static constexpr bool SATURATES = BLOB_PI_SATURATES != 0;
+    static constexpr bool HANDS_ON = true;
     const RecB* __restrict__ rec;
     const double* __restrict__ rho_s;
     const RecSelf* __restrict__ selfr;
     RecBC* bc;
     double *Pi, *BwOut;
+    double *va, *vh;
+    unsigned char* marks;
+    __device__ __forceinline__ bool hands_on() const { return marks != nullptr; }
+    __device__ __forceinline__ void hand_on(int b, bool any_live) const { marks[b] = any_live ? 1 : 0; }
     struct Row { Q4 r0, rv; double rho_i, cs_i, ms_i, h_i; };
     struct Nb { Q8 q; double rho; };
     __device__ __forceinline__ BlobSides sides() const { return {rho_s, 1}; }
@@ -276,19 +287,25 @@
     __device__ __forceinline__ Vel short_global(int j) const { return gload4(reinterpret_cast<const double*>(&rec[j]) + 4); }
     __device__ __forceinline__ static Vel short_none(const Row& r) { return r.rv; }
     __device__ __forceinline__ static double term_short(const Vel& qv, const Row& r) { return pi_rel(qv, r.rv); }
-    __device__ __forceinline__ u64 finish(const Sums& a, double maxrel, const Row& r, int i, int o) const {
+    __device__ __forceinline__ u64 finish(const Sums& a, double maxrel, const Row& r, int i, int o, bool has_first,
+                                          bool& live) const {
         Pi[o] = a.pi;
         const double bw = fmax(r.ms_i, 0.0) * a.pi;
         bc[i].Bw = bw;
         if (BwOut) BwOut[o] = bw;
+        if (marks) {
+            live = !sphx_row_settled(bw, has_first, true);
+            if (!live) visc_settle_store(va, vh, o);
+        }
         return (r.ms_i > 0.0) ? ct_vote_bits(r.h_i, maxrel) : SPHX_CT_NONE;
     }
 };
 BLOB_KERNEL blob_pi_kernel(BLOB_COMMON, const int* __restrict__ omap, int n_active, const RecB* __restrict__ recb,
                            const double* __restrict__ rho_s, const RecSelf* __restrict__ selfr, RecBC* bc, double* Pi,
-                           double* BwOut, u64* ct_bits, BlobSel sel, u64* counts) {
-    blob_pass(PiPass{recb, rho_s, selfr, bc, Pi, BwOut}, n, npad, k, nblk, nbr, slot16, uniq, qorder, 0, omap, n_active,
-              ct_bits, sel, counts);
+                           double* BwOut, u64* ct_bits, BlobSel sel, u64* counts, double* va, double* vh,
+                           unsigned char* marks) {
+    blob_pass(PiPass{recb, rho_s, selfr, bc, Pi, BwOut, va, vh, marks}, n, npad, k, nblk, nbr, slot16, uniq, qorder, 0, omap,
+              n_active, ct_bits, sel, counts);
 }
 
 struct ViscPass {
@@ -301,6 +318,7 @@
     const RecBC* __restrict__ bc;
     const double* __restrict__ m;
     double *va, *vh;
+    bool handed;
     struct Row { Q4 r0, rv; double hi2, ci, Bi, mi; };
     struct Nb { Q8 q; double c1; };
     __device__ __forceinline__ BlobSides sides() const {
@@ -337,16 +355,84 @@
     }
     __device__ __forceinline__ double own(int i) const { return bc[i].Bw; }
     __device__ __forceinline__ void settle(int o) const {
-        const double q = __builtin_nan("");
-        va[3 * (size_t)o + 0] = q; va[3 * (size_t)o + 1] = q; va[3 * (size_t)o + 2] = q;
-        vh[o] = q;
+        if (!handed) visc_settle_store(va, vh, o);
     }
 };
+#define VISC_NONE (-2)
+#define VISC_ROUND (16 * PASS_T)
+__device__ __forceinline__ int visc_own_blobs(const unsigned char* __restrict__ marks, int nblk, int& total) {
+    __shared__ int wave_tot[PASS_T / 64];
+    const int lane = threadIdx.x & 63, wv = threadIdx.x >> 6;
+    auto marked = [&](int b0, unsigned (&w)[4]) -> int {
+        w[0] = w[1] = w[2] = w[3] = 0u;
+        if (b0 >= nblk) return 0;
+        const uint4 mk = *reinterpret_cast<const uint4*>(marks + b0);
+        w[0] = mk.x; w[1] = mk.y; w[2] = mk.z; w[3] = mk.w;
+        int cnt = 0;
+#pragma unroll
+        for (int q = 0; q < 16; ++q) {
+            if (b0 + q >= nblk) w[q >> 2] &= ~(0xFFu << (8 * (q & 3)));
+            cnt += ((w[q >> 2] >> (8 * (q & 3))) & 0xFFu) ? 1 : 0;
+        }
+        return cnt;
+    };
+    unsigned w[4];
+    int mine = 0;
+    for (int base = 0; base < nblk; base += VISC_ROUND) mine += marked(base + 16 * (int)threadIdx.x, w);
+    mine = wave_scan_incl(mine);
+    if (lane == 63) wave_tot[wv] = mine;
+    __syncthreads();
+    total = 0;
+#pragma unroll
+    for (int q = 0; q < PASS_T / 64; ++q) total += wave_tot[q];
+    if (total == 0) return VISC_NONE;
+    if (total == nblk) return -1;
+    int before = 0;
+    for (int base = 0; base < nblk; base += VISC_ROUND) {
+        __syncthreads();
+        const int b0 = base + 16 * (int)threadIdx.x;
+        const int cnt = marked(b0, w);
+        const int incl = wave_scan_incl(cnt);
+        if (lane == 63) wave_tot[wv] = incl;
+        __syncthreads();
+        int r = before + incl - cnt;
+#pragma unroll
+        for (int q = 0; q < PASS_T / 64; ++q) {
+            const int tw = wave_tot[q];
+            if (q < wv) r += tw;
+            before += tw;
+        }
+        if (cnt) {
+#pragma unroll
+            for (int q = 0; q < 16; ++q) {
+                if ((w[q >> 2] >> (8 * (q & 3))) & 0xFFu) {
+                    const int bi = xcd_block_inv(r, total);
+                    if (bi % (int)gridDim.x == (int)blockIdx.x) blob_own_list()[bi / (int)gridDim.x] = b0 + q;
+                    ++r;
+                }
+            }
+        }
+    }
+    __syncthreads();
+    return ((int)blockIdx.x < total) ? (total - 1 - (int)blockIdx.x) / (int)gridDim.x + 1 : 0;
+}
+
 BLOB_KERNEL blob_visc_kernel(BLOB_COMMON, int clip, const int* __restrict__ omap, int n_active,
                              const RecB* __restrict__ recb, const RecBC* __restrict__ bc, const double* __restrict__ m,
-                             double* va, double* vh, BlobSel sel, u64* counts) {
-    blob_pass(ViscPass{recb, bc, m, va, vh}, n, npad, k, nblk, nbr, slot16, uniq, qorder, clip, omap, n_active, nullptr, sel,
-              counts);
+                             double* va, double* vh, BlobSel sel, u64* counts,
+                             const unsigned char* __restrict__ marks) {
+    int own_n = -1;
+    if (marks) {
+        int total;
+        own_n = visc_own_blobs(marks, nblk, total);
+        if (counts && blockIdx.x == 0 && threadIdx.x == 0) {
+            atomicAdd(counts + BLOB_CNT_BLOBS_SETTLED, (u64)(nblk - total));
+            if (own_n == VISC_NONE) atomicAdd(counts + BLOB_CNT_LAUNCHES_SKIPPED, (u64)1);
+        }
+        if (own_n == VISC_NONE) return;
+    }
+    blob_pass(ViscPass{recb, bc, m, va, vh, marks != nullptr}, n, npad, k, nblk, nbr, slot16, uniq, qorder, clip, omap, n_active,
+              nullptr, sel, counts, own_n);
 }
 
 struct ViscPwPass {
@@ -723,17 +809,29 @@
                        sphx_blob_sel(ctx, ctx->pass_part));
 }
 
-int sphx_blob_pi(sphx_ctx* ctx, int64_t n, int k, u64* ct_bits) {
+bool sphx_blob_can_hand_visc(sphx_ctx* ctx, int64_t n) {
+    if (!ctx->qorder || !ctx->blob_lists || ctx->map_perm || ctx->blob_split_valid) return false;
+    const int nblk = (int)((sphx_pad64(n) + BLOB_P - 1) / BLOB_P);
+    return nblk <= BLOB_OWN_MAX * sphx_blob_grid(ctx, nblk);
+}
+int sphx_blob_size_marks(sphx_ctx* ctx, int64_t n) {
+    const size_t nblk = (size_t)((sphx_pad64(n) + BLOB_P - 1) / BLOB_P);
+    return sphx_ensure(ctx, ctx->visc_live, (nblk + 15) / 16 * 16);
+}
+
+int sphx_blob_pi(sphx_ctx* ctx, int64_t n, int k, u64* ct_bits, bool hand_on) {
     return blob_launch(ctx, blob_pi_kernel, PiPass::PER_SLOT, 0, n, k, ctx->map_perm, blob_n_active(ctx, n), ctx->recv.as<RecB>(),
                        ctx->rho_s.as<double>(), ctx->self_s.as<RecSelf>(), ctx->bc_s.as<RecBC>(), ctx->Pi.as<double>(),
                        ctx->map_perm ? ctx->Bw.as<double>() : nullptr, ct_bits, sphx_blob_sel(ctx, ctx->pass_part),
-                       ctx->scal.as<u64>() + SC_SETTLED);
-}
-
-int sphx_blob_visc(sphx_ctx* ctx, int64_t n, int k, const double* m) {
+                       ctx->scal.as<u64>() + SC_SETTLED, hand_on ? ctx->va.as<double>() : nullptr,
+                       hand_on ? ctx->vh.as<double>() : nullptr, hand_on ? ctx->visc_live.as<unsigned char>() : nullptr);
+}
+
+int sphx_blob_visc(sphx_ctx* ctx, int64_t n, int k, const double* m, bool handed) {
     return blob_launch(ctx, blob_visc_kernel, ViscPass::PER_SLOT, 0, n, k, ctx->clip_grad, ctx->map_perm, blob_n_active(ctx, n),
                        ctx->recv.as<RecB>(), ctx->bc_s.as<RecBC>(), m, ctx->va.as<double>(), ctx->vh.as<double>(),
-                       sphx_blob_sel(ctx, ctx->pass_part), ctx->scal.as<u64>() + SC_SETTLED);
+                       sphx_blob_sel(ctx, ctx->pass_part), ctx->scal.as<u64>() + SC_SETTLED,
+                       handed ? ctx->visc_live.as<const unsigned char>() : nullptr);
 }
 
 int sphx_blob_visc_pw(sphx_ctx* ctx, int64_t n, int k, const double* m, u64* ct_bits) {
diff --git a/sph-code_amd/csrc/sphx_internal.h b/sph-code_amd/csrc/sphx_internal.h
--- a/sph-code_amd/csrc/sphx_internal.h
+++ b/sph-code_amd/csrc/sphx_internal.h
@@ -287,6 +287,7 @@
     DevBuf tie_list;
     DevBuf slot16, uniq;
     DevBuf blob_class, blob_split;
+    DevBuf visc_live;
     DevBuf rho, rhod, nden, G, Pi, Bw, va, vh, ha, F;
     DevBuf scal;
     DevBuf cell_of, cell_start, cell_fill, perm, inv, scan_tmp, bbox_tmp;
@@ -353,6 +354,12 @@
     const int q = nb >> 3, r = nb & 7, x = b & 7, s = b >> 3;
     return x * q + (x < r ? x : r) + s;
 }
+__device__ __forceinline__ int xcd_block_inv(int p, int nb) {
+    const int q = nb >> 3, r = nb & 7, head = r * (q + 1);
+    const int x = p < head ? p / (q + 1) : r + (p - head) / q;
+    const int s = p < head ? p % (q + 1) : (p - head) % q;
+    return s * 8 + x;
+}
 
 #ifndef SPHX_SUM_PARTS
 #define SPHX_SUM_PARTS 4
@@ -386,7 +393,7 @@
     SC_DENSEP = 14,
     SC_KGDBG = 16,
     SC_SETTLED = 24,
-    SC_NSLOTS = 26
+    SC_NSLOTS = 27
 };
 
 enum {
@@ -457,8 +464,8 @@
 int sphx_blob_density_species(sphx_ctx* ctx, int64_t n, int k, bool lean, int S, const double* fun, const int* row_of,
                               const double* m_sorted, double* F, double* Z, double* agb, int agb_on);
 int sphx_blob_density(sphx_ctx* ctx, int64_t n, int k, bool lean);
-int sphx_blob_pi(sphx_ctx* ctx, int64_t n, int k, u64* ct_bits);
-int sphx_blob_visc(sphx_ctx* ctx, int64_t n, int k, const double* m);
+int sphx_blob_pi(sphx_ctx* ctx, int64_t n, int k, u64* ct_bits, bool hand_on);
+int sphx_blob_visc(sphx_ctx* ctx, int64_t n, int k, const double* m, bool handed);
 int sphx_blob_visc_pw(sphx_ctx* ctx, int64_t n, int k, const double* m, u64* ct_bits);
 int sphx_blob_species(sphx_ctx* ctx, int64_t n, int k, int S, const double* fun, const int* row_of, const double* m_sorted, double* F,
                       double* Z, double* agb, int agb_on);
@@ -536,8 +543,10 @@
 };
 int sphx_prep(sphx_ctx* ctx, int64_t n, const PrepIn& in, bool pairwise, hipStream_t stream);
 int sphx_pass_density(sphx_ctx* ctx, int64_t n, int k, bool lean = false);
-int sphx_pass_pi(sphx_ctx* ctx, int64_t n, int k, const double* h, const double* ptype);
-int sphx_pass_visc(sphx_ctx* ctx, int64_t n, int k, const double* m);
+bool sphx_blob_can_hand_visc(sphx_ctx* ctx, int64_t n);
+int sphx_blob_size_marks(sphx_ctx* ctx, int64_t n);
+int sphx_pass_pi(sphx_ctx* ctx, int64_t n, int k, const double* h, const double* ptype, bool hand_visc = false);
+int sphx_pass_visc(sphx_ctx* ctx, int64_t n, int k, const double* m, bool hand_visc = false);
 int sphx_pass_visc_pw(sphx_ctx* ctx, int64_t n, int k, const double* m);
 int sphx_pass_species(sphx_ctx* ctx, int64_t n, int k, int s, const double* fun, double* F);
 int sphx_step_species(sphx_ctx* ctx, int64_t n, int k);
diff --git a/sph-code_amd/csrc/sphx_sums.hip b/sph-code_amd/csrc/sphx_sums.hip
--- a/sph-code_amd/csrc/sphx_sums.hip
+++ b/sph-code_amd/csrc/sphx_sums.hip
@@ -209,14 +209,14 @@
     block_min_vote<256>(my_ct, ct_bits);
 }
 
-int sphx_pass_pi(sphx_ctx* ctx, int64_t n, int k, const double* h, const double* ptype) {
+int sphx_pass_pi(sphx_ctx* ctx, int64_t n, int k, const double* h, const double* ptype, bool hand_visc) {
     (void)ptype; (void)h;
     SPHX_TRY(sphx_ensure(ctx, ctx->Pi, (size_t)n * sizeof(double)));
     SPHX_TRY(sphx_ensure(ctx, ctx->Bw, (size_t)n * sizeof(double)));
     u64* ct = ctx->scal.as<u64>() + SC_CT_BITS;
     if (!ctx->ct_primed) SPHX_TRY(sphx_prime_ct(ctx, ct));
     ctx->ct_primed = false;
-    if (ctx->qorder && ctx->blob_lists) return sphx_blob_pi(ctx, n, k, ct);
+    if (ctx->qorder && ctx->blob_lists) return sphx_blob_pi(ctx, n, k, ct, hand_visc);
     hipLaunchKernelGGL(pass_pi_kernel, dim3((unsigned)((n + 255) / 256)), dim3(256), 0, ctx->stream,
                        (int)n, (int)sphx_pad64(n), k, ctx->nbr.as<int>(), ctx->recv.as<RecB>(),
                        ctx->rho_s.as<double>(), ctx->self_s.as<RecSelf>(), ctx->bc_s.as<RecBC>(), ctx->qorder,
@@ -270,10 +270,10 @@
     vh[o] = heat * m[o] / 2.0;
 }
 
-int sphx_pass_visc(sphx_ctx* ctx, int64_t n, int k, const double* m) {
+int sphx_pass_visc(sphx_ctx* ctx, int64_t n, int k, const double* m, bool hand_visc) {
     SPHX_TRY(sphx_ensure(ctx, ctx->va, (size_t)n * 3 * sizeof(double)));
     SPHX_TRY(sphx_ensure(ctx, ctx->vh, (size_t)n * sizeof(double)));
-    if (ctx->qorder && ctx->blob_lists) return sphx_blob_visc(ctx, n, k, m);
+    if (ctx->qorder && ctx->blob_lists) return sphx_blob_visc(ctx, n, k, m, hand_visc);
     hipLaunchKernelGGL(pass_visc_kernel, dim3((unsigned)((n + 255) / 256)), dim3(256), 0, ctx->stream,
                        (int)n, (int)sphx_pad64(n), k, ctx->clip_grad, ctx->nbr.as<int>(), ctx->recv.as<RecB>(),
                        ctx->bc_s.as<RecBC>(), ctx->qorder,
```

New measurement: 960.0 million, median of 6. +1.9%, better.
